# dvalcarce/filmyou-core

Hardware: AMD Instinct MI355X
Metric: top-N recs/sec (RM2), ml25m shape (higher is better)
Workload: dtype f32 (scores and logs fp32 / v_log_f32, folded in fp64; co-rating sums 64-bit fixed point in LDS (fp64 fallback); G stored as 24-bit e7m17 floats scaled per cluster above 4096 items; ratings fp16 in the row kernel when exactly representable)

## Files before the change

### filmyou-core_amd/csrc/fy_api.hip

```cpp
#include <algorithm>
#include <cstdlib>
#include <memory>
#include <mutex>
#include <new>
#include <unordered_map>

#include "fy_prep.hpp"
#include "fy_rm2.hpp"
#include "fy_ratings_update.hpp"
#include "fy_rm2_request.hpp"
#include "fy_itemsim_request.hpp"

namespace fy {
static thread_local char g_err[512] = "";
void set_error(const char* fmt, ...) {
    va_list ap;
    va_start(ap, fmt);
    vsnprintf(g_err, sizeof g_err, fmt, ap);
    va_end(ap);
}
const char* last_error() { return g_err; }
}

using namespace fy;

void fy::load_tuning_from_env(Tuning& t) {
    t = Tuning{};
    if (const char* e = getenv("FY_M24")) t.pack24 = atoi(e) != 0;
    if (const char* e = getenv("FY_M24_MIN_ITEMS")) t.pack24_min_items = std::max(0, atoi(e));
    if (const char* e = getenv("FY_SCORE_SLICES")) t.max_slices = atoi(e);
    if (const char* e = getenv("FY_SCORE_UPW")) { int v = atoi(e); if (v >= 1) t.users_per_wave = v; }
    if (const char* e = getenv("FY_PRUNE")) t.prune = atoi(e) != 0;
    if (const char* e = getenv("FY_LAZY_MIRROR")) t.lazy_mirror = atoi(e) != 0;
    if (const char* e = getenv("FY_REFINE")) t.refine = atoi(e) != 0;
    if (const char* e = getenv("FY_REFINE_C")) { double v = atof(e); if (v >= 0.0 && v < 1e6) t.refine_c = (float)v; }
    if (const char* e = getenv("FY_FULL_WALK_SPARSE")) t.full_walk_sparse = atoi(e) != 0;
    if (const char* e = getenv("FY_PREP_PACKED")) t.prep_packed = atoi(e) != 0;
    if (const char* e = getenv("FY_OVERLAP_VALUES")) t.overlap_values = atoi(e) != 0;
    if (const char* e = getenv("FY_SHARD_PREP")) t.shard_prep = atoi(e) != 0;
    if (const char* e = getenv("FY_SUP_BOUNDS")) t.sup_bounds = atoi(e) != 0;
    if (const char* e = getenv("FY_COOP")) t.coop = atoi(e) != 0;
    if (const char* e = getenv("FY_COOP_FORCE")) t.coop_force = atoi(e) != 0;
    if (const char* e = getenv("FY_COOC_PK")) t.cooc_pk = atoi(e) != 0;
    if (const char* e = getenv("FY_COOC_F32")) t.cooc_f32 = atoi(e) != 0;
    if (const char* e = getenv("FY_COOC_HALF")) t.cooc_half = atoi(e) != 0;
    if (const char* e = getenv("FY_COOC_FX")) t.cooc_fx = atoi(e) != 0;
    if (const char* e = getenv("FY_PANEL_MIN_CLUSTERS")) { int v = atoi(e); if (v >= 1) t.panel_min_clusters = v; }
    if (const char* e = getenv("FY_PANEL_COLS")) { int v = atoi(e); if (v >= 256) { t.panel_cols = v; t.panel_wide_below_users = 0; } }
    if (const char* e = getenv("FY_PANEL_WIDE_BELOW_USERS")) { int v = atoi(e); if (v >= 0) t.panel_wide_below_users = v; }
    if (const char* e = getenv("FY_PANEL_MAX_CH")) { int v = atoi(e); if (v >= 256) t.panel_max_ch = v; }
    if (const char* e = getenv("FY_BOUNDED_TABLES")) t.bounded_tables = atoi(e) != 0;
    if (const char* e = getenv("FY_COOC_PLANES")) t.cooc_planes = atoi(e) != 0;
    if (const char* e = getenv("FY_SCORE_HEAVY")) { int v = atoi(e); if (v >= 0) t.score_heavy = v; }
    if (const char* e = getenv("FY_PANEL_REPAIR")) t.panel_repair = atoi(e) != 0;
    if (const char* e = getenv("FY_PANEL_MULTI_LAUNCH")) t.panel_multi_launch = atoi(e) != 0;
    if (const char* e = getenv("FY_FLAT")) t.flat_batch = atoi(e) != 0;
    if (const char* e = getenv("FY_PANEL_SYM")) t.panel_sym = atoi(e) != 0;
    if (const char* e = getenv("FY_DEBUG_SYNC")) t.debug_sync = atoi(e);
    if (const char* e = getenv("FY_PANEL_GROUP_MB")) t.panel_group_bytes = std::max<int64_t>(0, (int64_t)atoll(e)) << 20;
    if (const char* e = getenv("FY_FLAT_BUDGET_MB")) t.flat_budget = std::max<int64_t>(0, (int64_t)atoll(e)) << 20;
    if (const char* e = getenv("FY_PANEL_TWO_PHASE")) t.panel_two_phase = atoi(e) != 0;
    if (const char* e = getenv("FY_PANEL_LANES")) { int v = atoi(e); if (v >= 1 && v <= 8) t.panel_lanes = v; }
    if (const char* e = getenv("FY_PRUNE_MIN_ITEMS")) { t.prune_min_items = atoi(e); t.prune_min_users = 0; }
    if (const char* e = getenv("FY_PRUNE_MIN_USERS")) { int v = atoi(e); if (v >= 0) t.prune_min_users = v; }
    if (const char* e = getenv("FY_SEED_CHUNKS")) { int v = atoi(e); if (v >= 0 && v <= 40) { t.seed_chunks = v; t.seed_forced = v > 0; } }
    if (const char* e = getenv("FY_WORKSPACE_GB")) { long v = atol(e); if (v >= 1) t.workspace_default = (int64_t)v << 30; }
    if (const char* e = getenv("FY_LANES")) { int v = atoi(e); if (v >= 1 && v <= 8) { t.lanes = v; t.lanes_forced = true; } }
    if (const char* e = getenv("FY_COOC_BLOCK")) { int v = atoi(e); if (v == 256 || v == 512 || v == 1024) t.cooc_block = v; }
    if (const char* e = getenv("FY_COOC_MAX_CH")) { int v = atoi(e); if (v >= 64 && v <= 20224) { t.cooc_max_ch = v; t.cooc_max_ch_forced = true; } }
    if (const char* e = getenv("FY_TOPN_FORCE_SELECT")) t.force_select = atoi(e) != 0;
    if (const char* e = getenv("FY_MAX_SURV_FRAC")) { double v = atof(e); if (v >= 0.0) t.max_surv_frac = v; }
    if (const char* e = getenv("FY_REQ_FULL_SHARE")) { double v = atof(e); if (v >= 0.0) t.req_full_share = v; }
    if (const char* e = getenv("FY_REQ_CHUNK")) { int v = atoi(e); if (v >= 64 && v <= 16384 && v % 64 == 0) t.req_chunk = v; }
    if (const char* e = getenv("FY_UPD_LDS_KEYS")) { int v = atoi(e); if (v >= 0 && v <= fy::UPD_LDS_KEYS_MAX) t.upd_lds_keys = v; }
    if (const char* e = getenv("FY_ISIM_HEAVY")) t.isim_heavy = std::max(0, atoi(e));
    if (const char* e = getenv("FY_ISIM_GRAM")) t.isim_gram = atoi(e) != 0;
    if (const char* e = getenv("FY_ISIM_GRAM_MIN_ITEMS")) t.isim_gram_min_items = std::max(0, atoi(e));
    if (const char* e = getenv("FY_ISIM_CAPG")) { int v = atoi(e); if (v >= 1 && v <= 2040) t.isim_capg = v; }
    if (const char* e = getenv("FY_ISIM_ACC32")) t.isim_acc32 = atoi(e) != 0;
    if (const char* e = getenv("FY_ISIM_PIECE")) { int v = atoi(e); if (v >= 64 && v <= 8192 && v % 64 == 0) t.isim_piece = v; }
    if (const char* e = getenv("FY_ISIM_REQ_CHUNK")) { int v = atoi(e); if (v >= 64 && v <= 16384 && v % 64 == 0) t.isim_req_chunk = v; }
    if (const char* e = getenv("FY_ISIM_REQ_ROWS")) t.isim_req_rows = std::max(0, atoi(e));
}

namespace {
std::mutex& g_jobs_mu = *new std::mutex;
std::unordered_map<const fy_rm2_job*, fy::Context*>& g_jobs = *new std::unordered_map<const fy_rm2_job*, fy::Context*>;
fy::Context* job_context(const fy_rm2_job* j) {
    std::lock_guard<std::mutex> g(g_jobs_mu);
    auto it = g_jobs.find(j);
    return it == g_jobs.end() ? nullptr : it->second;
}
inline void select_device(const fy::Context* ctx) {
    if (ctx) FY_HIP(hipSetDevice(ctx->device));
}
}

#define FY_TRY try {
#define FY_CATCH                                                           \
    }                                                                      \
    catch (const fy::Failure& f) { return f.code; }                        \
    catch (const std::bad_alloc&) {                                        \
        fy::set_error("host allocation failed");                           \
        return FY_ERR_OUT_OF_MEMORY;                                       \
    }                                                                      \
    catch (const std::exception& e) {                                      \
        fy::set_error("unexpected: %s", e.what());                         \
        return FY_ERR_HIP;                                                 \
    }                                                                      \
    return FY_OK;

extern "C" {

int fy_abi_version(void) { return FY_ABI_VERSION; }
const char* fy_last_error(void) { return fy::last_error(); }

int fy_context_create(int device_ordinal, fy_context** out) {
    if (!out) { set_error("out is NULL"); return FY_ERR_INVALID_ARGUMENT; }
    *out = nullptr;
    FY_TRY
    int n = 0;
    hipError_t e = hipGetDeviceCount(&n);
    if (e != hipSuccess || n <= 0) {
        (void)hipGetLastError();
        FY_FAIL(FY_ERR_NO_DEVICE, "no HIP device is visible (%s); this library has no CPU fallback",
                e == hipSuccess ? "device count 0" : hipGetErrorString(e));
    }
    if (device_ordinal < 0 || device_ordinal >= n) FY_FAIL(FY_ERR_INVALID_ARGUMENT, "device %d of %d", device_ordinal, n);
    FY_HIP(hipSetDevice(device_ordinal));
    hipDeviceProp_t prop;
    FY_HIP(hipGetDeviceProperties(&prop, device_ordinal));
    if (std::string(prop.gcnArchName).rfind("gfx950", 0) != 0)
        FY_FAIL(FY_ERR_NO_DEVICE, "device %d is %s; the kernels are built for gfx950 (MI355X) only", device_ordinal, prop.gcnArchName);
    std::unique_ptr<fy_context> c(new fy_context);
    c->c.device = device_ordinal;
    c->c.num_cus = prop.multiProcessorCount;
    c->c.total_mem = prop.totalGlobalMem;
    FY_HIP(hipStreamCreateWithFlags(&c->c.stream, hipStreamNonBlocking));
    fy::load_tuning_from_env(c->c.tune);
    *out = c.release();
    FY_CATCH
}

void fy_context_destroy(fy_context* c) {
    if (!c) return;
    (void)hipSetDevice(c->c.device);
    if (c->c.stream) {
        for (hipStream_t x : c->c.aux) (void)hipStreamSynchronize(x);
        (void)hipStreamSynchronize(c->c.stream);
        c->c.trim();
        for (auto& kv : c->c.capacity) (void)hipFree(kv.first);
        c->c.capacity.clear();
        for (hipStream_t x : c->c.aux) { (void)hipStreamSynchronize(x); (void)hipStreamDestroy(x); }
        (void)hipStreamDestroy(c->c.stream);
    }
    delete c;
}

int fy_context_inject_alloc_failure(fy_context* c, int64_t nth) {
    if (!c || nth < 0) { set_error("context is NULL or nth < 0"); return FY_ERR_INVALID_ARGUMENT; }
    c->c.fail_alloc_in = nth;
    return FY_OK;
}

int fy_context_reload_tuning(fy_context* c) {
    if (!c) { set_error("context is NULL"); return FY_ERR_INVALID_ARGUMENT; }
    fy::load_tuning_from_env(c->c.tune);
    return FY_OK;
}

int fy_context_synchronize(fy_context* c) {
    if (!c) { set_error("context is NULL"); return FY_ERR_INVALID_ARGUMENT; }
    FY_TRY
    select_device(&c->c);
    FY_HIP(hipStreamSynchronize(c->c.stream));
    FY_CATCH
}

void* fy_context_stream(fy_context* c) { return c ? (void*)c->c.stream : nullptr; }

int fy_ratings_create(fy_context* c, int64_t nnz, const int32_t* user, const int32_t* item, const float* score, int location,
                      fy_ratings** out) {
    if (!out) { set_error("out is NULL"); return FY_ERR_INVALID_ARGUMENT; }
    *out = nullptr;
    if (!c) { set_error("context is NULL"); return FY_ERR_INVALID_ARGUMENT; }
    if (nnz < 0 || (nnz > 0 && (!user || !item || !score))) { set_error("ratings arrays are NULL or nnz < 0"); return FY_ERR_INVALID_ARGUMENT; }
    if (location != FY_HOST && location != FY_DEVICE) { set_error("location must be FY_HOST or FY_DEVICE"); return FY_ERR_INVALID_ARGUMENT; }
    FY_TRY
    FY_HIP(hipSetDevice(c->c.device));
    std::unique_ptr<fy_ratings> r(new fy_ratings);
    r->ctx = &c->c;
    r->nnz = nnz;
    r->user.alloc(&c->c, (size_t)nnz);
    r->item.alloc(&c->c, (size_t)nnz);
    r->score.alloc(&c->c, (size_t)nnz);
    if (nnz) {
        const hipMemcpyKind k = location == FY_HOST ? hipMemcpyHostToDevice : hipMemcpyDeviceToDevice;
        FY_HIP(hipMemcpyAsync(r->user.get(), user, (size_t)nnz * 4, k, c->c.stream));
        FY_HIP(hipMemcpyAsync(r->item.get(), item, (size_t)nnz * 4, k, c->c.stream));
        FY_HIP(hipMemcpyAsync(r->score.get(), score, (size_t)nnz * 4, k, c->c.stream));
        FY_HIP(hipStreamSynchronize(c->c.stream));
        fy::ratings_id_bounds(&c->c, r.get());
    }
    *out = r.release();
    FY_CATCH
}
// ... 349 lines not shown
```

### filmyou-core_amd/csrc/fy_rm2.hip

```cpp
#include <algorithm>
#include <cmath>
#include <cstdlib>
#include <type_traits>

#include "fy_cooc.hpp"
#include "fy_prep.hpp"
#include <chrono>
#include "fy_rm2.hpp"
#include "fy_rm2_plan.hpp"
#include "fy_rm2_request.hpp"

namespace fy {

static inline int grid_for(int64_t n, int block = 256, int cap = 256 * 16) {
    int64_t g = ceil_div(n, block);
    return (int)std::max<int64_t>(1, std::min<int64_t>(g, cap));
}

constexpr int PAIR_HEAVY = 2048;
struct PairPass {
    const int32_t* __restrict__ rank_pair;
    const int32_t* __restrict__ pair_start;
    const int32_t* __restrict__ pair_di;
    const int32_t* __restrict__ csc_slot;
// ... 964 lines not shown
        }
        best = max(max(best, max(v[0], v[1])), max(v[2], v[3]));
    }
    if (Bmax_) {
        uint8_t* bp = reinterpret_cast<uint8_t*>(Bmax_) + ((int64_t)row * ldb + B) * 3;
        bp[0] = (uint8_t)best;
        bp[1] = (uint8_t)(best >> 8);
        bp[2] = (uint8_t)(best >> 16);
    }
}

__global__ __launch_bounds__(256) void k_mirror_diag(float* __restrict__ M_, int64_t ldm, int32_t Ic, float* __restrict__ Bmax_, int64_t ldb) {
    mirror_diag_body(M_, ldm, Ic, Bmax_, ldb);
}
struct PanelDesc {
    float* Gp;
    float* Bmax64;
    uint32_t* Brep;
    int64_t panel_cols, ldb64;
    int32_t Ic, p_eff, nsub, pad;
};
__global__ __launch_bounds__(1024) void k_mirror_tiles_multi(const PanelDesc* __restrict__ D) {
    const PanelDesc d = D[blockIdx.z];
    if ((int)blockIdx.x >= (int)(d.panel_cols / 128) || (int)blockIdx.y >= (int)(d.panel_cols / 256) - 1) return;
    mirror_tiles_body(d.Gp, d.panel_cols, d.p_eff, nullptr, 0);
}
__global__ __launch_bounds__(256) void k_mirror_diag_multi(const PanelDesc* __restrict__ D) {
    const PanelDesc d = D[blockIdx.y];
    if ((int)blockIdx.x >= (int)(d.panel_cols / 256)) return;
    mirror_diag_body(d.Gp, d.panel_cols, d.p_eff, nullptr, 0);
}
__global__ __launch_bounds__(256) void k_panel_colmax(const PanelDesc* __restrict__ D) {
    const PanelDesc dsc = D[blockIdx.z];
    const float* __restrict__ Gp_ = dsc.Gp;
    float* __restrict__ Bmax64_ = dsc.Bmax64;
    uint32_t* __restrict__ Brep = dsc.Brep;
    const int64_t panel_cols = dsc.panel_cols, ldb64 = dsc.ldb64;
    const int32_t Ic = dsc.Ic, p_eff = dsc.p_eff, nsub = dsc.nsub;
    if ((int)blockIdx.x * 256 >= p_eff || (int)blockIdx.y * 16 >= nsub) return;
    __shared__ uint32_t sh_m[16][257], sh_r[16][257];
    const int lane = threadIdx.x & 63, wave = threadIdx.x >> 6;
    const int col0 = blockIdx.x * 256, sbg = blockIdx.y * 16;
    const int c = col0 + 4 * lane;
    const unsigned char* __restrict__ base = reinterpret_cast<const unsigned char*>(Gp_) + (int64_t)c * 3;
    const int64_t pitch = panel_cols * 3;
    for (int s = 0; s < 4; s++) {
        const int sb = sbg + 4 * wave + s;
        uint32_t t1[4] = {0, 0, 0, 0}, t2[4] = {0, 0, 0, 0};
        if (sb < nsub) {
            const int j0 = 64 * sb, nr = min(64, Ic - j0);
            for (int r = 0; r < nr; r += 8) {
                uint32_t d[8][3];
#pragma unroll
                for (int x = 0; x < 8; x++) {
                    const uint32_t* __restrict__ p = reinterpret_cast<const uint32_t*>(base + (int64_t)(j0 + min(r + x, nr - 1)) * pitch);
                    d[x][0] = p[0]; d[x][1] = p[1]; d[x][2] = p[2];
                }
#pragma unroll
                for (int x = 0; x < 8; x++) {
                    if (r + x < nr) {
                        uint32_t v[4];
                        fy_unpack24_raw(d[x][0], d[x][1], d[x][2], v);
#pragma unroll
                        for (int q = 0; q < 4; q++) {
                            const uint32_t key = (v[q] << 6) | (uint32_t)(r + x);
                            t2[q] = max(min(t1[q], key), t2[q]);
                            t1[q] = max(t1[q], key);
                        }
                    }
                }
            }
        }
#pragma unroll
        for (int q = 0; q < 4; q++) {
            sh_m[4 * wave + s][4 * lane + q] = t1[q] >> 6;
            sh_r[4 * wave + s][4 * lane + q] = (t1[q] >> 6) ? (((t2[q] >> 6) << 8) | (t1[q] & 63u)) : 0u;
        }
    }
    __syncthreads();
    const int i = col0 + threadIdx.x;
    if (i < p_eff) {
        uint32_t m[16];
#pragma unroll
        for (int k = 0; k < 16; k++) m[k] = sh_m[k][threadIdx.x];
        uint32_t* __restrict__ bp = reinterpret_cast<uint32_t*>(reinterpret_cast<unsigned char*>(Bmax64_) + ((int64_t)i * ldb64 + sbg) * 3);
#pragma unroll
        for (int g = 0; g < 4; g++) {
            const uint32_t* v = m + 4 * g;
            bp[3 * g + 0] = v[0] | (v[1] << 24);
            bp[3 * g + 1] = (v[1] >> 8) | (v[2] << 16);
            bp[3 * g + 2] = (v[2] >> 16) | (v[3] << 8);
        }
        uint32_t* __restrict__ rp = Brep + (int64_t)i * ldb64 + sbg;
#pragma unroll
        for (int k = 0; k < 16; k++) rp[k] = sh_r[k][threadIdx.x];
    }
}

static void launch_mirror(Context* ctx, float* M, int64_t ldm, int32_t Ic, float* Bmax, int64_t ldb, hipStream_t st, const int32_t* need = nullptr,
                          int32_t write_below = 0x7FFFFFFF, bool diag = true) {
    const int nblk = (int)(ldm / 256), ntile = (int)(ldm / 128);
    if (nblk > 1) {
        FY_HIP(hipFuncSetAttribute(reinterpret_cast<const void*>(k_mirror_tiles), hipFuncAttributeMaxDynamicSharedMemorySize, 128 * MIRROR_PITCH));
        const bool split = !need && Bmax && write_below < nblk - 1;
        const int ny = split ? write_below : nblk - 1;
        if (ny > 0) {
            k_mirror_tiles<<<dim3(ntile, ny), 1024, 128 * MIRROR_PITCH, st>>>(M, ldm, Ic, Bmax, ldb, need, write_below);
            FY_KERNEL_CHECK();
        }
        if (split) {
            k_colmax_upper<<<dim3(nblk, nblk - 1 - write_below), 1024, 0, st>>>(M, ldm, Ic, Bmax, ldb, write_below);
            FY_KERNEL_CHECK();
        }
    }
    if (diag) {
        k_mirror_diag<<<nblk, 256, 0, st>>>(M, ldm, Ic, Bmax, ldb);
        FY_KERNEL_CHECK();
    }
}

static void cooc_rm2_allow_lds() {
    const int bytes = 160 * 1024 - 256;
    FY_HIP(hipFuncSetAttribute(reinterpret_cast<const void*>(k_cooc_rm2<false, double>), hipFuncAttributeMaxDynamicSharedMemorySize, bytes));
    FY_HIP(hipFuncSetAttribute(reinterpret_cast<const void*>(k_cooc_rm2<true, double>), hipFuncAttributeMaxDynamicSharedMemorySize, bytes));
    FY_HIP(hipFuncSetAttribute(reinterpret_cast<const void*>(k_cooc_rm2<false, float>), hipFuncAttributeMaxDynamicSharedMemorySize, bytes));
    FY_HIP(hipFuncSetAttribute(reinterpret_cast<const void*>(k_cooc_rm2<true, float>), hipFuncAttributeMaxDynamicSharedMemorySize, bytes));
    FY_HIP(hipFuncSetAttribute(reinterpret_cast<const void*>(k_cooc_rm2<true, unsigned long long>), hipFuncAttributeMaxDynamicSharedMemorySize, bytes));
    FY_HIP(hipFuncSetAttribute(reinterpret_cast<const void*>(k_cooc_rm2<true, uint32_t>), hipFuncAttributeMaxDynamicSharedMemorySize, bytes));
    FY_HIP(hipFuncSetAttribute(reinterpret_cast<const void*>(k_cooc_rm2<true, unsigned long long, 1>), hipFuncAttributeMaxDynamicSharedMemorySize, bytes));
    FY_HIP(hipFuncSetAttribute(reinterpret_cast<const void*>(k_cooc_rm2_multi<true, unsigned long long, 0>), hipFuncAttributeMaxDynamicSharedMemorySize, bytes));
    FY_HIP(hipFuncSetAttribute(reinterpret_cast<const void*>(k_cooc_rm2_multi<true, unsigned long long, 1>), hipFuncAttributeMaxDynamicSharedMemorySize, bytes));
}
static void stray_allow_lds();

#include "fy_rm2_kernels.hpp"

static_assert(TOPN_MAX == fy::TOPN_LIST_MAX, "fy_rm2.hpp states the top-N kernels' limit for the other translation units");
static void stray_allow_lds() {
    FY_HIP(hipFuncSetAttribute(reinterpret_cast<const void*>(k_score_stray), hipFuncAttributeMaxDynamicSharedMemorySize, (STRAY_UCAP + 1) * (int)sizeof(int32_t)));
}

void launch_topn_rows(Context* ctx, hipStream_t st, const float* S, int64_t ldS, int32_t n_cols, int32_t n_rows,
                      const int32_t* n_out, const int32_t* out_off, const int32_t* rank_item_raw, const int32_t* slot2du,
                      const int32_t* uid, int32_t slot0, int32_t aux_value, int32_t* out_user, int32_t* out_item,
                      float* out_score, int32_t* out_aux, int32_t* overflow, int32_t* any_overflow, int32_t top_n_hint) {
    if (n_rows <= 0) return;
    if (!st) st = ctx->stream;
    TopNArgs TA{S, ldS, n_cols, n_out, out_off, rank_item_raw, slot2du, uid, slot0, slot0, aux_value, out_user, out_item, out_score, out_aux,
                0, 0, nullptr, nullptr, 0, nullptr, nullptr, nullptr};
    FY_HIP(hipMemsetAsync(any_overflow, 0, sizeof(int32_t), st));
    if (top_n_hint > TOPN_LONG) k_topn_long<<<n_rows, 256, (size_t)fy_topn_long_cap(top_n_hint) * 8, st>>>(TA, overflow, any_overflow, 0, fy_topn_long_cap(top_n_hint));
    else k_topn_fast<<<n_rows, 256, 0, st>>>(TA, overflow, any_overflow, 0);
    FY_KERNEL_CHECK();
    k_topn_select<<<n_rows, 256, 0, st>>>(TA, overflow, any_overflow);
    FY_KERNEL_CHECK();
}

}

using namespace fy;

struct TableCache {
    bool valid = false;
    int64_t total_segments = 0;
    std::vector<int32_t> sig;
    bool have_x = false;
    DevBuf<float> csc_x, csc_x_over_s;
    DevBuf<uint32_t> csr_pk, y_pk;
    DevBuf<int32_t> csc_rank, samples;
    std::vector<SegTable> segs, segs_tail;
    DevBuf<int32_t> g_co, g_co_tail, g_cnt, g_ptr, g_start;
    DevBuf<int2> g_seg;
    DevBuf<float> g_w;
};
struct RM2Static {
    int32_t K = 0, rank = 0, world = 1;
    int32_t max_item = -1;
    bool has_count = false;
    std::vector<int32_t> map_user, map_cluster, cluster_count;
    Prepared P;
    int32_t slot_lo = 0, slot_hi = 0;
    DevBuf<double> partial;
    bool sharded = false;
    int64_t n_raw_users = 0, n_raw_items = 0;
    std::vector<int32_t> owner;
    DevBuf<double> partial_raw;
    int deferred_code = 0;
    std::string deferred_msg;
    int64_t exchange_len() const { return sharded ? n_raw_items + 1 + n_raw_users + 1 : (int64_t)P.nI + 1; }
    DevBuf<double> b_rank, usum_slot;
    DevBuf<long long> walk_rank;
    DevBuf<int32_t> cnt_rank, deg_slot;
    DevBuf<float> fx_rank;
    std::vector<float> fx_bounds;
    double ms_build = 0;
    TableCache tables;
    std::shared_ptr<void> request_state;
    bool matches(const fy_rm2_params* prm, int64_t n_map, const int32_t* mu, const int32_t* mc, const int32_t* cc) const {
        if (K != prm->number_of_clusters || rank != prm->rank || world != prm->world || (int64_t)map_user.size() != n_map || has_count != (cc != nullptr)) return false;
        if (n_map && (memcmp(map_user.data(), mu, (size_t)n_map * 4) || memcmp(map_cluster.data(), mc, (size_t)n_map * 4))) return false;
        if (cc && memcmp(cluster_count.data(), cc, (size_t)K * 4)) return false;
        return true;
    }
};

struct fy_rm2_job {
    Context* ctx = nullptr;
    fy_rm2_params prm{};
    std::shared_ptr<RM2Static> S;
    Prepared& P;
    int32_t &slot_lo, &slot_hi;
    DevBuf<double>& partial;
    DevBuf<double> stats;
    DevBuf<double> stats_raw;
    bool have_global = false;
    double ms_prepare = 0;
    bool from_cache = false;
    fy_collectives coll{};
    bool have_coll = false;
    DevBuf<double> gathered;
    DevBuf<double>&b_rank, &usum_slot;
    DevBuf<long long>& walk_rank;
    DevBuf<int32_t>&cnt_rank, &deg_slot;
    DevBuf<float>& fx_rank;
    std::vector<float>& fx_bounds;
    bool count_balanced = false;
    explicit fy_rm2_job(std::shared_ptr<RM2Static> s)
        : S(std::move(s)), P(S->P), slot_lo(S->slot_lo), slot_hi(S->slot_hi), partial(S->partial), b_rank(S->b_rank), usum_slot(S->usum_slot),
          walk_rank(S->walk_rank), cnt_rank(S->cnt_rank), deg_slot(S->deg_slot), fx_rank(S->fx_rank), fx_bounds(S->fx_bounds) {}
};

static void owner_range(const fy_rm2_job* J, int k, int32_t& lo, int32_t& hi) {
    if (J->S->sharded) { lo = 0; hi = k == J->prm.rank ? J->P.nU : 0; return; }
    if (!J->count_balanced) { rank_slot_range(J->P, k, J->prm.world, lo, hi); return; }
    const int64_t n = J->P.nU, W = J->prm.world;
    lo = (int32_t)(n * k / W);
    hi = (int32_t)(n * (k + 1) / W);
}

using ScoreTune = fy::Tuning;


static int cooc_item_grab(int64_t visits, int64_t n_items) { return n_items > 0 && visits / n_items < 12000 ? 8 : 1; }

static void launch_cooc_rm2(Context* ctx, const ScoreTune& tune, bool use_pk, const CoocArgs& CA_, const MEpilogue& ME, int n_items,
                            int32_t* counter, hipStream_t st) {
    if (n_items <= 0) return;
    CoocArgs CA = CA_;
    CA.acc_quarter = tune.cooc_planes ? cooc_lds_columns(CA.CH) / 4 : 0;
    const bool acc32 = CA.acc32 && use_pk && CA.fx_scale > 0.0 && !tune.cooc_f32;
    const size_t lds = (size_t)cooc_lds_columns(CA.CH) * ((tune.cooc_f32 || acc32) ? 4 : 8);
    const int by_lds = (int)std::max<size_t>(1, (160 * 1024 - 512) / (lds + 64));
    int block = tune.cooc_block;
    if (!block) block = by_lds >= 4 ? 256 : (by_lds >= 2 ? 512 : 1024);
    const int per_cu = std::max(1, std::min(by_lds, 2048 / block));
    const int grid = std::min(n_items, ctx->num_cus * per_cu);
    if (acc32) {
        k_cooc_rm2<true, uint32_t><<<grid, block, lds, st>>>(CA, ME, n_items, counter);
    } else if (use_pk && CA.fx_scale > 0.0 && !tune.cooc_f32) {
        if (ME.ceil24) k_cooc_rm2<true, unsigned long long, 1><<<grid, block, lds, st>>>(CA, ME, n_items, counter);
        else k_cooc_rm2<true, unsigned long long><<<grid, block, lds, st>>>(CA, ME, n_items, counter);
    } else if (!tune.cooc_f32) {
        if (use_pk) k_cooc_rm2<true, double><<<grid, block, lds, st>>>(CA, ME, n_items, counter);
        else k_cooc_rm2<false, double><<<grid, block, lds, st>>>(CA, ME, n_items, counter);
    } else {
        if (use_pk) k_cooc_rm2<true, float><<<grid, block, lds, st>>>(CA, ME, n_items, counter);
        else k_cooc_rm2<false, float><<<grid, block, lds, st>>>(CA, ME, n_items, counter);
    }
    FY_KERNEL_CHECK();
}

bool fy::gram_half_build(Context* ctx, const Prepared& P, const float* csc_w, const float* bounds3, float* G, int64_t ldm, double* ms_tables,
                         double* ms_walk, const float* csr_ones) {
    const ScoreTune tune = ctx->tune;
    const int32_t Ic = P.nP;
    if (P.K != 1 || (!csr_ones && (!P.ratings_fp16_exact || !P.ratings_positive)) || Ic <= 0) return false;
    int fxk = fx_exponent(bounds3);
    if (fxk < 0) return false;
    const int m = csr_ones ? 0 : P.ratings_frac_bits;
    const bool acc32 = tune.isim_acc32 && m <= 4 && (double)bounds3[2] * bounds3[2] * std::ldexp(1.0, 2 * m) < 16777216.0 &&
                       (double)bounds3[0] * bounds3[2] * std::ldexp(1.0, 2 * m) < 4294967296.0;
    if (acc32) fxk = 2 * m;
    int32_t CH, nch;
    pick_chunks(Ic, acc32 && !tune.cooc_max_ch_forced ? 2 * tune.cooc_max_ch : tune.cooc_max_ch, CH, nch);
    if (nch >= 256) return false;
    hipStream_t st = ctx->stream;
    cooc_rm2_allow_lds();
    EventTimer t_tab(ctx), t_walk(ctx);
    const size_t s0 = t_tab.begin();
    DevBuf<uint32_t> csr_pk(ctx, (size_t)P.nnz);
    k_pack_csr<<<grid_for(P.nnz), 256, 0, st>>>(0, (int32_t)P.nnz, CH, P.csr_idx.get(), csr_ones ? csr_ones : P.csr_r.get(), csr_pk.get());
    FY_KERNEL_CHECK();
    DevBuf<int32_t> co(ctx, (size_t)P.nU * (nch + 1)), csc_rank(ctx, (size_t)P.nnz);
    build_chunk_offsets(ctx, P.rowptr.get(), P.csr_idx.get(), 0, P.nU, CH, nch, co.get(), st);
    k_csc_rank<<<grid_for(P.nnz), 256, 0, st>>>(P.nnz, P.csc_pair.get(), P.pair_rank.get(), csc_rank.get());
    FY_KERNEL_CHECK();
    SegTable segs;
    DevBuf<int32_t> samples;
    build_csr_samples(ctx, P.nnz, P.csr_idx.get(), samples, st);
    build_segments(ctx, P.csc_slot.get(), csc_w, co.get(), 0, 0, (int32_t)P.nnz, nch, segs, st, csc_rank.get(), P.csr_idx.get(), CH, nullptr, 0, 0, samples.get());
    CoocArgs CA{P.rank_pair.get(), P.pair_start.get(), segs.ptr.get(), segs.seg.get(), segs.w.get(), P.csr_idx.get(), nullptr, 0, 0, Ic, CH, nch,
                0, Ic, 0, (int32_t)P.nnz, nullptr, 0, csr_pk.get(), nullptr, (uint32_t)std::min<int64_t>((int64_t)P.nnz * 4, 0xFFFFFFFFll)};
    CA.half = 1;
    CA.fx_scale = std::ldexp(1.0, fxk);
    CA.acc32 = acc32 ? 1 : 0;
    const int n_items = (int)cooc_item_count(Ic, CH, nch, true);
    DevBuf<int2> item_seg(ctx, (size_t)Ic * nch);
// ... 634 lines not shown
        build_segments(ctx, P.csc_slot.get(), tc.csc_x_over_s.get(), co, p.sbase, p.q0, p.nq, 1, tc.segs_tail[pi], ts, nullptr, nullptr, 0,
                       tc.csc_rank.get(), p.p_eff, 0);
    }
}

static void build_job_tables(fy_rm2_job* J, const JobPlan& jp, bool tables_cached, std::vector<int32_t>& csr_range, std::vector<DevBuf<int32_t>>& co_lane) {
    Context* ctx = J->ctx;
    const Prepared& P = J->P;
    hipStream_t st = ctx->stream;
    TableCache& tc = J->S->tables;
    const std::vector<Plan>& plans = jp.plans;
    if (!tables_cached) {
        tc.valid = false;
        tc.segs.clear();
        tc.segs_tail.clear();
        tc.segs.resize(plans.size());
        tc.segs_tail.resize(plans.size());
        tc.csr_pk.alloc(ctx, jp.use_pk ? (size_t)P.nnz : 1);
        tc.y_pk.alloc(ctx, jp.any_tail ? (size_t)P.nnz : 1);
        tc.csc_rank.alloc(ctx, jp.any_half ? (size_t)P.nnz : 1);
        if (jp.any_half) {
            k_csc_rank<<<grid_for(P.nnz), 256, 0, st>>>(P.nnz, P.csc_pair.get(), P.pair_rank.get(), tc.csc_rank.get());
            FY_KERNEL_CHECK();
            build_csr_samples(ctx, P.nnz, P.csr_idx.get(), tc.samples, st);
        }
    }
    csr_range.assign(2 * plans.size() + 2, 0);
    {
        std::vector<int32_t> where(2 * plans.size());
        for (size_t pi = 0; pi < plans.size(); pi++) {
            where[2 * pi] = plans[pi].sbase;
            where[2 * pi + 1] = plans[pi].sbase + plans[pi].Uc;
        }
        gather_to_host_i32(ctx, P.rowptr.get(), where, csr_range.data());
    }
    const bool all_at_once = plans.size() > 1 && !jp.any_coop;
    co_lane.resize((size_t)jp.NS);
    if (!all_at_once)
        for (auto& b : co_lane) b.alloc(ctx, jp.co_all);
    if (tables_cached) return;
    if (all_at_once) build_tables_all(ctx, P, plans, csr_range, jp.use_pk, tc, st);
    else
        for (size_t pi = 0; pi < plans.size(); pi++) build_tables(J, jp, pi, csr_range, st, co_lane[0].get());
}

struct FlatBuffers {
    DevBuf<char> flatM;
    DevBuf<float> flatS;
    DevBuf<int2> flat_seg;
    DevBuf<int32_t> flat_id, flat_ov, flat_flags, flat_cnt;
    DevBuf<CoocLaunch> d_flat_launch;
    DevBuf<FlatDesc> d_flat[2];
};
static void score_flat_batches(const ScoreShared& X, FlatBuffers& F) {
    fy_rm2_job* J = X.J;
    Context* ctx = X.J->ctx;
    const Prepared& P = X.J->P;
    fy_result* R = X.R;
    const ScoreTune& tune = *X.tune;
    const fy_rm2_params& prm = X.J->prm;
    const JobPlan& jp = *X.jp;
    hipStream_t st = ctx->stream;
    TableCache& tc = J->S->tables;
    const int32_t lo = X.lo;
    const double lambda = prm.lambda;
    constexpr int VEC = 4;
    for (size_t first = 0; first < jp.plans.size();) {
        std::vector<CoocLaunch> fb;
        std::vector<FlatDesc> fd[2];
        SyncOnUnwind fb_fd_guard(st);
        size_t m_bytes = 0, s_el = 0, i_el = 0, u_el = 0, n_flat = 0, last = first;
        int64_t batch_bytes = 0;
        for (; last < jp.plans.size(); last++) {
            const Plan& p = jp.plans[last];
            if (!p.flat) continue;
            if (n_flat && batch_bytes + flat_need(p) > jp.flat_budget) break;
            batch_bytes += flat_need(p);
            m_bytes += round_up((int64_t)p.Ic * p.ldm * (p.pack24 ? 3 : 4), 256);
            s_el += (size_t)(p.b - p.a) * p.ldm;
            i_el += (size_t)p.Ic * p.nch;
            u_el += (size_t)(p.b - p.a);
            n_flat++;
        }
        if (n_flat) {
            F.flatM.alloc(ctx, m_bytes);
            F.flatS.alloc(ctx, s_el);
            F.flat_seg.alloc(ctx, i_el);
            F.flat_id.alloc(ctx, i_el);
            F.flat_ov.alloc(ctx, u_el);
            F.flat_flags.alloc(ctx, 2 * n_flat);
            size_t m_at = 0, s_at = 0, i_at = 0, u_at = 0, k = 0;
            int max_grid[2] = {0, 0}, max_users[2] = {0, 0};
            for (size_t pi = first; pi < last; pi++) {
                const Plan& p = jp.plans[pi];
                if (!p.flat) continue;
                const int c = p.c;
                const int32_t nb = p.b - p.a;
                float* const Mc = reinterpret_cast<float*>(F.flatM.get() + m_at);
                float* const Sc = F.flatS.get() + s_at;
                CoocArgs CA{P.rank_pair.get(), P.pair_start.get(), tc.segs[pi].ptr_(), tc.segs[pi].seg_(), tc.segs[pi].w_(), P.csr_idx.get(),
                            X.csr_x, p.pbase, p.sbase, p.Ic, p.CH, p.nch, 0, p.Ic, p.q0, p.nq, nullptr, 0, X.csr_pk, nullptr,
                            (uint32_t)std::min<int64_t>((int64_t)P.nnz * 4, 0xFFFFFFFFll)};
                const int fxk = fx_exponent(&J->fx_bounds[3 * (size_t)c]);
                CA.fx_scale = std::ldexp(1.0, fxk);
                const double w2s = (1.0 - lambda) * (1.0 - lambda) * (double)X.gscale[(size_t)c];
                MEpilogue ME{Mc, p.ldm, (float)w2s, std::ldexp(w2s, -fxk), p.pack24 ? 1 : 0, nullptr, p.ldb, 0, 0, nullptr, p.ldb64, nullptr};
                const int n_items = (int)cooc_item_count(p.Ic, p.CH, p.nch, false);
                CA.item_seg = F.flat_seg.get() + i_at;
                CA.item_id = F.flat_id.get() + i_at;
                CA.item_grab = cooc_item_grab((size_t)c < P.cluster_deg2.size() ? P.cluster_deg2[c] : P.sum_deg2, n_items);
                fb.push_back(CoocLaunch{CA, ME, n_items, 0});

                const int n_chunks = (int)ceil_div(p.Ic, 64 * VEC);
                const int64_t fill = ceil_div(8 * (int64_t)ctx->num_cus, (int64_t)std::max(1, n_chunks) * (int64_t)n_flat);
                const int n_slices = (int)std::max<int64_t>(1, std::min<int64_t>(tune.max_slices, std::min<int64_t>(ceil_div(nb, 4), std::max<int64_t>(ceil_div(nb, 4 * (int64_t)tune.users_per_wave), fill))));
                FlatDesc d{};
                ScoreArgs& SA = d.SA;
                SA.M = Mc; SA.ldm = p.ldm; SA.Ic = p.Ic; SA.a_rank = X.a_rank + p.pbase; SA.b_rank = X.b_rank + p.pbase;
                SA.rb_off = P.rowptr.get() + p.sbase;
                SA.csr_idx = P.csr_idx.get(); SA.csr_e = X.csr_e; SA.csr_q = X.csr_q;
                SA.pvpi = X.pvpi; SA.n_out = X.n_out; SA.slot_lo = lo; SA.slot_base = p.sbase; SA.slot0 = p.a; SA.n_users = nb;
                SA.S = Sc; SA.ldS = p.ldm; SA.n_slices = n_slices; SA.n_chunks = n_chunks;
                d.n_heavy = F.flat_flags.get() + 2 * k;
                d.any_overflow = F.flat_flags.get() + 2 * k + 1;
                SA.n_heavy = tune.score_heavy > 0 ? d.n_heavy : nullptr;
                d.heavy_thresh = tune.score_heavy > 0 ? std::min(tune.score_heavy, 32) : 0x7FFFFFFF;
                d.TA = TopNArgs{Sc, p.ldm, p.Ic, X.n_out, X.out_off, P.rank_item_raw.get() + p.pbase, P.slot2du.get(), P.uid.get(), lo, p.a, c,
                                R->d_key0.get(), R->d_key1.get(), R->d_value.get(), R->d_aux.get(), 0, 0, nullptr, nullptr, 0, nullptr, nullptr, nullptr};
                d.overflow = F.flat_ov.get() + u_at;
                d.score_grid = n_chunks * n_slices;
                d.n_users = nb;
                const int f = p.pack24 ? 1 : 0;
                max_grid[f] = std::max(max_grid[f], d.score_grid);
                max_users[f] = std::max(max_users[f], nb);
                fd[f].push_back(d);
                m_at += (size_t)round_up((int64_t)p.Ic * p.ldm * (p.pack24 ? 3 : 4), 256);
                s_at += (size_t)nb * p.ldm;
                i_at += (size_t)p.Ic * p.nch;
                u_at += (size_t)nb;
                k++;
            }
            const size_t sp = X.t_cooc->begin(st);
            launch_cooc_rm2_multi(ctx, tune, fb, false, F.d_flat_launch, F.flat_cnt, st, true);
            X.t_cooc->end(sp, st);
            R->st.cooc_launches++;
            for (int f = 0; f < 2; f++) {
                if (fd[f].empty()) continue;
                const unsigned ny = (unsigned)fd[f].size();
                F.d_flat[f].alloc(ctx, fd[f].size());
                FY_HIP(hipMemcpyAsync(F.d_flat[f].get(), fd[f].data(), fd[f].size() * sizeof(FlatDesc), hipMemcpyHostToDevice, st));
                const size_t ss = X.t_score->begin(st);
                k_count_heavy_multi<<<(ny + 63) / 64, 64, 0, st>>>(F.d_flat[f].get(), (int32_t)ny);
                FY_KERNEL_CHECK();
                if (f) k_score_multi<4, true, 8><<<dim3((unsigned)max_grid[f], ny), 256, 0, st>>>(F.d_flat[f].get(), P.csr_idx.get(), X.csr_e, X.csr_q, X.pvpi, X.n_out);
                else k_score_multi<4, false, 8><<<dim3((unsigned)max_grid[f], ny), 256, 0, st>>>(F.d_flat[f].get(), P.csr_idx.get(), X.csr_e, X.csr_q, X.pvpi, X.n_out);
                FY_KERNEL_CHECK();
                X.t_score->end(ss, st);
                R->st.score_launches++;
                const size_t tt = X.t_topn->begin(st);
                k_topn_fast_multi<<<dim3((unsigned)max_users[f], ny), 256, 0, st>>>(F.d_flat[f].get(), tune.force_select);
                FY_KERNEL_CHECK();
                k_topn_select_multi<<<dim3((unsigned)max_users[f], ny), 256, 0, st>>>(F.d_flat[f].get(), X.prune_counters + 2);
                FY_KERNEL_CHECK();
                X.t_topn->end(tt, st);
            }
            FY_HIP(hipStreamSynchronize(st));
        }
        first = last;
    }
}

struct PanelBuf {
    DevBuf<float> Gp, Bmax64, amax64, bmax64;
    DevBuf<uint32_t> Brep;
    DevBuf<double> head32, tail32;
};
struct PanelPtrs {
    float *Gp, *Bmax64;
    uint32_t* Brep;
    float *amax64, *bmax64;
};
struct PanelSet {
    std::vector<PanelBuf> pbuf;
    std::vector<Lane> plane;
    std::vector<CoocLaunch> batch_main, batch_tail;
    DevBuf<CoocLaunch> d_batch_main, d_batch_tail;
    DevBuf<int32_t> d_cnt_main, d_cnt_tail;
    DevBuf<PanelDesc> d_panel_desc;
    std::vector<PanelDesc> hpd;
};
static void group_buffers(Context* ctx, const JobPlan& jp, int seed_chunks, const std::vector<Lane>& lanes, int grp, PanelSet& PS) {
    const std::vector<Plan>& plans = jp.plans;
    std::vector<PanelBuf>& pbuf = PS.pbuf;
    std::vector<Lane>& plane = PS.plane;
    for (size_t pi = 0; pi < plans.size(); pi++) {
        const Plan& p = plans[pi];
        if (!p.panel || jp.group_of[pi] != grp) continue;
        pbuf[pi].Gp.alloc(ctx, (size_t)p.Ic * p.panel_cols * 3 / 4 + 4);
        pbuf[pi].Bmax64.alloc(ctx, (size_t)p.Ic * p.ldb64 * 3 / 4 + 4);
        pbuf[pi].Brep.alloc(ctx, (size_t)p.Ic * p.ldb64 + 4);
        pbuf[pi].amax64.alloc(ctx, (size_t)p.ldb64);
        pbuf[pi].bmax64.alloc(ctx, (size_t)p.ldb64);
    }
    for (size_t pi = 0; pi < plans.size(); pi++) {
        const Plan& p = plans[pi];
        if (!p.panel || jp.group_of[pi] != grp) continue;
        Lane& W = plane[pi];
        const size_t nbp = (size_t)(p.b - p.a);
        const size_t seed_cols = (size_t)std::min<int64_t>(ceil_div(p.Ic, 256), seed_chunks) * 256;
        W.st = lanes[pi % jp.NS].st;
        W.M.alloc(ctx, 1); W.Bmax.alloc(ctx, 1); W.amax.alloc(ctx, 1); W.bmax.alloc(ctx, 1);
        W.Gp.alloc(ctx, 1); W.Bmax64.alloc(ctx, 1); W.Brep.alloc(ctx, 1); W.amax64.alloc(ctx, 1); W.bmax64.alloc(ctx, 1);
        W.item_seg.alloc(ctx, (size_t)p.Ic * p.nch); W.item_id.alloc(ctx, (size_t)p.Ic * p.nch);
        W.item_seg_t.alloc(ctx, (size_t)std::max(1, p.Ic - p.p_eff)); W.item_id_t.alloc(ctx, (size_t)std::max(1, p.Ic - p.p_eff));
        W.S.alloc(ctx, nbp * seed_cols);
        W.overflow.alloc(ctx, nbp);
        W.any_overflow.alloc(ctx, 1);
        W.n_heavy.alloc(ctx, 1);
        W.UB.alloc(ctx, nbp * (size_t)p.ldb64);
        W.tau.alloc(ctx, nbp);
        W.surv.alloc(ctx, nbp * (size_t)p.ldb64);
        W.surv_mask.alloc(ctx, nbp * (size_t)p.ldb64);
        W.n_quads.alloc(ctx, nbp + 1);
        W.quad_prefix.alloc(ctx, nbp + 1);
    }
}

struct LaneGuard {
    Context* ctx;
    hipEvent_t fork = nullptr;
    int32_t* pinned = nullptr;
    ~LaneGuard() {
        for (hipStream_t x : ctx->aux) (void)hipStreamSynchronize(x);
        (void)hipStreamSynchronize(ctx->stream);
        if (fork) (void)hipEventDestroy(fork);
        if (pinned) (void)hipHostFree(pinned);
    }
};

struct ClusterVisit {
    size_t pi;
    int grp, phase;
    Lane* L;
    hipStream_t ls;
    PanelPtrs PP;
    DevBuf<double>*H32, *T32;
    Lane* own;
    PanelSet* PS;
    int32_t* pinned;
};
struct ClusterNumbers {
    int fxk;
    double w2s;
    bool refine;
    int32_t head_rows;
    int64_t ld_head;
};
static ClusterNumbers cluster_numbers(const ScoreShared& X, const Plan& p) {
    const fy_rm2_job* J = X.J;
    const ScoreTune& tune = *X.tune;
    const double lambda = J->prm.lambda;
    const int c = p.c;
    ClusterNumbers N{};
    N.fxk = (X.jp->use_pk && tune.cooc_fx && !J->fx_bounds.empty()) ? fx_exponent(&J->fx_bounds[3 * (size_t)c]) : -1;
    N.w2s = (1.0 - lambda) * (1.0 - lambda) * (double)X.gscale[(size_t)c];
    N.refine = tune.refine && p.pack24 && !p.coop && N.fxk >= 0 && J->S->max_item >= 0 && J->S->max_item < (1 << 28) && p.Ic >= 8;
    N.head_rows = (int32_t)std::min<int64_t>(p.Ic & ~3, std::max<int64_t>(256, std::min<int64_t>(1024, (int64_t)tune.seed_chunks * 256)));
    N.ld_head = p.psym ? (int64_t)p.p_eff : p.ldm;
    return N;
}
static void checkpoint(const ScoreShared& X, const ClusterVisit& V, const char* what) {
    if (X.tune->debug_sync != 1) return;
    const hipError_t e = hipDeviceSynchronize();
    fprintf(stderr, "[fy] group %d/%d phase %d plan %zu (cluster %d): %s -> %s\n", V.grp, X.jp->n_groups, V.phase, V.pi, X.jp->plans[V.pi].c, what, hipGetErrorString(e));
    fflush(stderr);
}

static void build_cluster_matrix(const ScoreShared& X, const ClusterVisit& V, const ClusterNumbers& N) {
    fy_rm2_job* J = X.J;
    Context* ctx = X.J->ctx;
    const Prepared& P = X.J->P;
    fy_result* R = X.R;
    const ScoreTune& tune = *X.tune;
    const JobPlan& jp = *X.jp;
    TableCache& tc = J->S->tables;
    const size_t pi = V.pi;
    const int phase = V.phase;
    const Plan& p = jp.plans[pi];
    Lane& L = *V.L;
    hipStream_t ls = V.ls;
    const PanelPtrs& PP = V.PP;
    const int c = p.c;
    const int32_t sbase = p.sbase, pbase = p.pbase, Ic = p.Ic, CH = p.CH, nch = p.nch;
    const int64_t ldm = p.ldm;
    const bool pack24 = p.pack24;
    const int fxk = N.fxk;
    const double w2s = N.w2s;
    CoocArgs CA{P.rank_pair.get(), P.pair_start.get(), tc.segs[pi].ptr_(), tc.segs[pi].seg_(), tc.segs[pi].w_(), P.csr_idx.get(),
                X.csr_x, pbase, sbase, Ic, CH, nch, 0, Ic, p.q0, p.nq, nullptr, 0, X.csr_pk, nullptr,
                (uint32_t)std::min<int64_t>((int64_t)P.nnz * 4, 0xFFFFFFFFll)};
    CA.fx_scale = fxk >= 0 ? std::ldexp(1.0, fxk) : 0.0;
    MEpilogue ME{L.M.get(), ldm, (float)w2s, fxk >= 0 ? std::ldexp(w2s, -fxk) : 0.0,
                 pack24 ? 1 : 0, (p.prune && !p.panel) ? L.Bmax.get() : nullptr, p.ldb, 0,
                 p.panel ? p.panel_cols : 0, p.panel ? PP.Bmax64 : nullptr, p.ldb64, p.panel ? PP.Brep : nullptr};
    if (p.panel) ME.M = PP.Gp;
    if (N.refine) {
        V.H32->alloc(ctx, (size_t)N.head_rows * N.ld_head + 4);
// ... 19 lines not shown
    const bool batched = phase == 1 && tune.panel_multi_launch && jp.use_pk && fxk >= 0 && !tune.cooc_f32;
    if (p.p_eff < Ic) {
        CoocArgs CB{P.rank_pair.get(), P.pair_start.get(), tc.segs_tail[pi].ptr_(), tc.segs_tail[pi].seg_(), tc.segs_tail[pi].w_(), P.csr_idx.get(),
                    X.csr_x, pbase, sbase, Ic, p.tail_width, 1, p.p_eff, Ic - p.p_eff, p.q0, p.nq, nullptr, 0, tc.y_pk.get(), nullptr, CA.pk_bytes};
        CB.fx_scale = CA.fx_scale;
        MEpilogue MB{reinterpret_cast<float*>(reinterpret_cast<char*>(PP.Bmax64) + (size_t)(p.p_eff / 64) * 3), p.tail_width, ME.w2, ME.fx_inv, 1,
                     nullptr, 0, 0, 0, nullptr, 0, nullptr, p.ldb64, 1};
        int2* const tseg = batched ? V.own->item_seg_t.get() : L.item_seg.get();
        int32_t* const tid = batched ? V.own->item_id_t.get() : L.item_id.get();
        if (!batched) {
            k_item_list<<<grid_for((int64_t)(Ic - p.p_eff)), 256, 0, ls>>>(CB, tseg, tid);
            FY_KERNEL_CHECK();
        }
        CB.item_seg = tseg;
        CB.item_id = tid;
        CB.item_grab = 8;
        if (batched) V.PS->batch_tail.push_back(CoocLaunch{CB, MB, Ic - p.p_eff, 0});
        else {
            FY_HIP(hipMemsetAsync(L.any_overflow.get(), 0, sizeof(int32_t), ls));
            launch_cooc_rm2(ctx, tune, jp.use_pk, CB, MB, Ic - p.p_eff, L.any_overflow.get(), ls);
            R->st.cooc_launches++;
        }
        CA.tail_row0 = p.p_eff;
        CA.tail_chunks = p.tail_chunks;
    }
    {
        CA.half = (p.half || p.psym) ? 1 : 0;
        if (p.psym) { CA.half_rows = p.p_eff; CA.head_chunks = p.tail_chunks; }
        const int n_items = p.psym ? (int)(cooc_half_item_index(p.p_eff - 1, p.tail_chunks - 1, CH, p.tail_chunks) + 1 + (int64_t)(Ic - p.p_eff) * p.tail_chunks)
                            : CA.tail_chunks > 0 ? (int)((int64_t)p.p_eff * nch + (int64_t)(Ic - p.p_eff) * p.tail_chunks)
                                                 : (int)cooc_item_count(Ic, CH, nch, p.half);
        int2* const mseg = batched ? V.own->item_seg.get() : L.item_seg.get();
        int32_t* const mid = batched ? V.own->item_id.get() : L.item_id.get();
        if (!batched) {
            k_item_list<<<grid_for((int64_t)Ic * nch), 256, 0, ls>>>(CA, mseg, mid);
            FY_KERNEL_CHECK();
        }
        CA.item_seg = mseg;
        CA.item_id = mid;
        CA.item_grab = cooc_item_grab(((size_t)c < P.cluster_deg2.size() ? P.cluster_deg2[c] : P.sum_deg2) / (p.half ? 2 : 1), n_items);
        if (batched) V.PS->batch_main.push_back(CoocLaunch{CA, ME, n_items, 0});
        else {
            FY_HIP(hipMemsetAsync(L.any_overflow.get(), 0, sizeof(int32_t), ls));
            launch_cooc_rm2(ctx, tune, jp.use_pk, CA, ME, n_items, L.any_overflow.get(), ls);
        }
    }
    X.t_cooc->end(sp, ls);
    X.side->join(ls);
    checkpoint(X, V, "row kernel queued / run");
    if (!batched) R->st.cooc_launches++;
    if (p.half) {
        const size_t sm = X.t_mirror->begin(ls);
        const bool lazy = p.prune && tune.lazy_mirror;
        launch_mirror(ctx, L.M.get(), ldm, Ic, p.prune ? L.Bmax.get() : nullptr, p.ldb, ls, nullptr, lazy ? std::min(tune.seed_chunks, p.nblk) : 0x7FFFFFFF);
        X.t_mirror->end(sm, ls);
    }
    if (p.prune && !p.panel && tune.sup_bounds && !jp.long_seed) {
        const int seed_b = std::min(tune.seed_chunks, p.nblk);
        std::vector<int32_t> first;
        sup_block_map(seed_b, p.nblk, first);
        const int n_sup = (int)first.size() - 1;
        first.resize(65, first.back());
        L.sup_first.alloc(ctx, 65);
        L.Bsup.alloc(ctx, (size_t)Ic * 64);
        L.asup.alloc(ctx, 64);
        L.bsupb.alloc(ctx, 64);
        FY_HIP(hipMemcpyAsync(L.sup_first.get(), first.data(), 65 * sizeof(int32_t), hipMemcpyHostToDevice, ls));
        FY_HIP(hipStreamSynchronize(ls));
        const size_t sb = X.t_score->begin(ls);
        k_build_bsup<<<std::min<int>((Ic + 3) / 4, ctx->num_cus * 32), 256, 0, ls>>>(Ic, n_sup, L.sup_first.get(), L.Bmax.get(), p.ldb, L.Bsup.get());
        FY_KERNEL_CHECK();
        k_sup_amax<<<1, 64, 0, ls>>>(n_sup, L.sup_first.get(), L.amax.get(), L.bmax.get(), L.asup.get(), L.bsupb.get());
        FY_KERNEL_CHECK();
        X.t_score->end(sb, ls);
    }
}

static void score_cluster(const ScoreShared& X, const ClusterVisit& V, const ClusterNumbers& N) {
    fy_rm2_job* J = X.J;
    Context* ctx = X.J->ctx;
    const Prepared& P = X.J->P;
    fy_result* R = X.R;
    const ScoreTune& tune = *X.tune;
    const fy_rm2_params& prm = X.J->prm;
    const JobPlan& jp = *X.jp;
    TableCache& tc = J->S->tables;
    const size_t pi = V.pi;
    const int phase = V.phase;
    const Plan& p = jp.plans[pi];
    Lane& L = *V.L;
    hipStream_t ls = V.ls;
    const PanelPtrs& PP = V.PP;
    const int c = p.c;
    const int32_t sbase = p.sbase, pbase = p.pbase, Ic = p.Ic, a = p.a, b = p.b;
    const int64_t ldm = p.ldm;
    const bool pack24 = p.pack24;
    const int32_t lo = X.lo;
    const double lambda = prm.lambda;
    const double w2s = N.w2s;
    const bool refine = N.refine;
    const int32_t head_rows = N.head_rows;
    const int64_t ld_head = N.ld_head;
    const DevBuf<double>&H32 = *V.H32, &T32 = *V.T32;
    constexpr int VEC = 4;
    const int64_t ldS = ldm, B = p.B;
    const int n_chunks = (int)ceil_div(Ic, 64 * VEC);
    const int32_t* row_off = P.rowptr.get() + sbase;
    auto score_args = [&](const float* Mx, int64_t ldmx, int32_t Icx, const float* ax, int32_t s0, int32_t nb, float* Sx, int64_t ldSx,
                          int n_slices, int nchunks) {
        ScoreArgs SA{};
        SA.M = Mx; SA.ldm = ldmx; SA.Ic = Icx; SA.a_rank = ax; SA.b_rank = X.b_rank + pbase; SA.rb_off = row_off;
        SA.csr_idx = P.csr_idx.get(); SA.csr_e = X.csr_e; SA.csr_q = X.csr_q;
        SA.pvpi = X.pvpi; SA.n_out = X.n_out; SA.slot_lo = lo; SA.slot_base = sbase; SA.slot0 = s0; SA.n_users = nb;
        SA.S = Sx; SA.ldS = ldSx; SA.n_slices = n_slices; SA.n_chunks = nchunks;
        if (tune.score_heavy > 0) {
            const int heavy = (int64_t)nb * nchunks < 8 * (int64_t)ctx->num_cus ? std::min(tune.score_heavy, 32) : tune.score_heavy;
            k_count_heavy<<<1, 64, 0, ls>>>(P.rowptr.get() + s0, nb, heavy, L.n_heavy.get());
            SA.n_heavy = L.n_heavy.get();
        }
        return SA;
    };
    auto refine_rows = [&](int32_t s0, int32_t nb) {
        if (!refine || nb <= 0) return;
        const size_t tt = X.t_topn->begin(ls);
        const int32_t n_ids = J->S->max_item + 1;
        L.colmap.alloc(ctx, (size_t)n_ids);
        FY_HIP(hipMemsetAsync(L.colmap.get(), 0xFF, (size_t)n_ids * sizeof(int32_t), ls));
        k_refine_colmap<<<(head_rows + 255) / 256, 256, 0, ls>>>(head_rows, P.rank_item_raw.get() + pbase, L.colmap.get());
        FY_KERNEL_CHECK();
        RefineArgs RA{};
        RA.slot0 = s0; RA.n_users = nb; RA.slot_lo = lo; RA.slot_base = sbase;
        RA.n_out = X.n_out; RA.out_off = X.out_off; RA.out_item = R->d_key1.get(); RA.out_score = R->d_value.get(); RA.out_item_w = R->d_key1.get();
        RA.rowptr = P.rowptr.get(); RA.csr_idx = P.csr_idx.get(); RA.csr_r = P.csr_r.get(); RA.usum_slot = J->usum_slot.get();
        RA.p_rank = X.p_rank + pbase; RA.b_rank = X.b_rank64 + pbase;
        RA.colmap = L.colmap.get(); RA.max_item = J->S->max_item;
        RA.head_rows = head_rows;
        RA.head32 = H32.get(); RA.ld_head = ld_head; RA.tail32 = p.psym ? T32.get() : nullptr; RA.tail_from = p.p_eff;
        if (!RA.head32 || (p.psym && !RA.tail32)) FY_FAIL(FY_ERR_STATE, "internal: cluster %d has no fp32 rows for the refinement pass", c);
        RA.unscale = 1.0 / (double)X.gscale[(size_t)c];
        RA.lambda = lambda; RA.ln_items = std::log((double)prm.number_of_items); RA.ln_users = std::log((double)p.Uc);
        RA.users_minus_1 = (double)(p.Uc - 1);
        RA.refine_c = tune.refine_c;
        RA.n_refined = X.prune_counters + 5;
        int lp2 = 64;
        while (lp2 < std::min<int>(prm.number_of_recommendations, Ic)) lp2 <<= 1;
        k_refine_rows<<<(nb + 3) / 4, 256, (size_t)4 * lp2 * sizeof(uint64_t), ls>>>(RA);
        FY_KERNEL_CHECK();
        X.t_topn->end(tt, ls);
    };
    auto full_pass = [&](int32_t s0, int32_t nb, float* Sx) {
        const int n_slices = score_slices(ctx->num_cus, tune, nb, n_chunks);
        ScoreArgs SA = score_args(L.M.get(), ldm, Ic, X.a_rank + pbase, s0, nb, Sx, ldS, n_slices, n_chunks);
        const size_t ss = X.t_score->begin(ls);
        if (pack24) k_score<4, true, 8><<<n_chunks * n_slices, 256, 0, ls>>>(SA.M, SA.a_rank, SA.rb_off, SA.csr_idx, SA.csr_e, SA.csr_q, SA.pvpi, SA.n_out, SA.S, SA);
        else k_score<4, false, 8><<<n_chunks * n_slices, 256, 0, ls>>>(SA.M, SA.a_rank, SA.rb_off, SA.csr_idx, SA.csr_e, SA.csr_q, SA.pvpi, SA.n_out, SA.S, SA);
        FY_KERNEL_CHECK();
        X.t_score->end(ss, ls);
        R->st.score_launches++;
        TopNArgs TA{Sx, ldS, Ic, X.n_out, X.out_off, P.rank_item_raw.get() + pbase, P.slot2du.get(), P.uid.get(), lo, s0, c,
                    R->d_key0.get(), R->d_key1.get(), R->d_value.get(), R->d_aux.get(), 0, 0, nullptr, nullptr, 0, nullptr, nullptr, nullptr};
        const size_t tt = X.t_topn->begin(ls);
        FY_HIP(hipMemsetAsync(L.any_overflow.get(), 0, sizeof(int32_t), ls));
        if (prm.number_of_recommendations > TOPN_LONG)
            k_topn_long<<<nb, 256, (size_t)fy_topn_long_cap(prm.number_of_recommendations) * 8, ls>>>(TA, L.overflow.get(), L.any_overflow.get(), tune.force_select,
                                                                                                 fy_topn_long_cap(prm.number_of_recommendations));
        else k_topn_fast<<<nb, 256, 0, ls>>>(TA, L.overflow.get(), L.any_overflow.get(), tune.force_select);
        FY_KERNEL_CHECK();
        k_topn_select<<<nb, 256, 0, ls>>>(TA, L.overflow.get(), L.any_overflow.get(), X.prune_counters + 2);
        FY_KERNEL_CHECK();
        X.t_topn->end(tt, ls);
        refine_rows(s0, nb);
    };
    for (int32_t s0 = a; s0 < b; s0 += (int32_t)B) {
        const int32_t nb = (int32_t)std::min<int64_t>(B, b - s0);
        if (!p.prune) { full_pass(s0, nb, L.S.get()); continue; }
        const int seed_chunks = std::min(n_chunks, tune.seed_chunks);
        const bool use_sup = tune.sup_bounds && !p.panel && !jp.long_seed;
        const int n_slices = score_slices(ctx->num_cus, tune, nb, seed_chunks + (use_sup ? 0 : (int)(p.ldb / 256)));
        const bool split = jp.two_phase && p.panel && s0 == sbase && nb == p.Uc;
        if (phase == 3 && !split) continue;
        size_t ss = X.t_score->begin(ls);
        const int seed_blocks = seed_chunks;
        const int64_t SC = (int64_t)seed_chunks * 256;
        const float* Gmat = p.panel ? PP.Gp : L.M.get();
        const int64_t gld = p.panel ? (int64_t)p.panel_cols : ldm;
        const int64_t bld = p.panel ? p.ldb64 : p.ldb;
        const int bchunks = (int)(bld / 256);
        int32_t hv[3] = {0, 0, 0};
        if (phase != 3) {
        if (use_sup) {
            ScoreArgs SU = score_args(Gmat, gld, Ic, X.a_rank + pbase, s0, nb, L.S.get(), SC, n_slices, seed_chunks);
            L.UBs.alloc(ctx, (size_t)nb * 64);
            SU.Bsup = L.Bsup.get(); SU.asup = L.asup.get(); SU.bsup_b = L.bsupb.get(); SU.UBsup = L.UBs.get();
            SU.n_sup = std::min(64, std::max(0, p.nblk - seed_chunks));
            k_score_sup<<<seed_chunks * n_slices, 256, 0, ls>>>(SU.M, SU.a_rank, SU.rb_off, SU.csr_idx, SU.csr_e, SU.csr_q, SU.pvpi, SU.n_out, SU.S, SU);
            FY_KERNEL_CHECK();
        }
        ScoreArgs SA = score_args(Gmat, gld, Ic, X.a_rank + pbase, s0, nb, L.S.get(), SC, n_slices, seed_chunks + bchunks);
        SA.chunks1 = seed_chunks;
        SA.M2 = p.panel ? PP.Bmax64 : L.Bmax.get();
        SA.ldm2 = bld;
        SA.Ic2 = p.panel ? p.nsub : p.nblk;
        SA.a2 = p.panel ? PP.amax64 : L.amax.get();
        SA.b2 = p.panel ? PP.bmax64 : L.bmax.get();
        SA.S2 = L.UB.get();
        SA.ldS2 = bld;
        SA.no_mask2 = 1;
        if (!use_sup) {
            k_score<4, true, 8><<<(seed_chunks + bchunks) * n_slices, 256, 0, ls>>>(SA.M, SA.a_rank, SA.rb_off, SA.csr_idx, SA.csr_e, SA.csr_q, SA.pvpi, SA.n_out, SA.S, SA);
            FY_KERNEL_CHECK();
        }
        TopNArgs T1{L.S.get(), SC, Ic, X.n_out, X.out_off, P.rank_item_raw.get() + pbase, P.slot2du.get(), P.uid.get(),
                    lo, s0, c, R->d_key0.get(), R->d_key1.get(), R->d_value.get(), R->d_aux.get(),
                    1, seed_chunks * 256, L.surv.get(), L.n_quads.get(), bld, L.tau.get()};
        if (jp.long_seed) {
            k_topn_long<<<nb, 256, (size_t)fy_topn_long_cap(prm.number_of_recommendations) * 8, ls>>>(T1, L.overflow.get(), L.any_overflow.get(), 0,
                                                                                                 fy_topn_long_cap(prm.number_of_recommendations));
        } else {
            int lp2 = 64;
            while (lp2 < std::min<int>(std::min<int>(Ic, seed_chunks * 256), TOPN_SAMPLE)) lp2 <<= 1;
            const unsigned sg = (unsigned)((nb + 3) / 4);
            if (lp2 <= 64) k_topn_seed<1><<<sg, 256, 0, ls>>>(T1, nb, L.overflow.get());
            else if (lp2 == 128) k_topn_seed<2><<<sg, 256, 0, ls>>>(T1, nb, L.overflow.get());
            else if (lp2 == 256) k_topn_seed<4><<<sg, 256, 0, ls>>>(T1, nb, L.overflow.get());
            else if (lp2 == 512) k_topn_seed<8><<<sg, 256, 0, ls>>>(T1, nb, L.overflow.get());
            else k_topn_seed<16><<<sg, 256, 0, ls>>>(T1, nb, L.overflow.get());
        }
        FY_KERNEL_CHECK();
        FY_HIP(hipMemsetAsync(L.n_quads.get(), 0, ((size_t)nb + 1) * sizeof(int32_t), ls));
        if (p.panel)
            k_bound_select_sub<<<grid_for((int64_t)nb * 64, 256), 256, 0, ls>>>(L.UB.get(), bld, p.nsub, p.nblk, seed_blocks, L.tau.get(),
                                                                               X.pvpi + (s0 - lo), nb, bld, L.surv.get(), L.surv_mask.get(), L.n_quads.get());
        else if (use_sup)
            k_bound_select_sup<<<grid_for((int64_t)nb * 64, 256), 256, 0, ls>>>(L.UBs.get(), std::min(64, std::max(0, p.nblk - seed_chunks)), L.sup_first.get(), L.tau.get(),
                                                                               X.pvpi + (s0 - lo), nb, p.ldb, L.surv.get(), L.n_quads.get());
        else
            k_bound_select<<<grid_for((int64_t)nb * 64, 256), 256, 0, ls>>>(L.UB.get(), p.ldb, p.nblk, seed_blocks, L.tau.get(), X.pvpi + (s0 - lo), nb,
                                                                           L.surv.get(), L.n_quads.get());
        FY_KERNEL_CHECK();
        if (tune.debug_sync == 3 && !p.panel) {
            DevBuf<int32_t> cnt(ctx, (size_t)p.nblk + 1);
            FY_HIP(hipMemsetAsync(cnt.get(), 0, ((size_t)p.nblk + 1) * sizeof(int32_t), ls));
            k_surv_block_counts<<<std::min<int>(nb, 4096), 64, 0, ls>>>(nb, L.n_quads.get(), L.surv.get(), p.ldb, cnt.get());
            std::vector<int32_t> hc((size_t)p.nblk + 1);
            FY_HIP(hipMemcpyAsync(hc.data(), cnt.get(), hc.size() * sizeof(int32_t), hipMemcpyDeviceToHost, ls));
            FY_HIP(hipStreamSynchronize(ls));
            int distinct = 0;
            long long total = 0;
            for (int b2 = 0; b2 < p.nblk; b2++) { distinct += hc[b2] > 0; total += hc[b2]; }
            fprintf(stderr, "[fy] cluster %d: %lld surviving (user, block) pairs in %d distinct blocks of %d:", c, total, distinct, p.nblk);
            for (int b2 = 0; b2 < p.nblk; b2++)
                if (hc[b2]) fprintf(stderr, " %d:%d", b2, hc[b2]);
            fprintf(stderr, "\n");
        }
        if (p.panel && tune.panel_repair) {
            RepairArgs RA{L.surv.get(), L.surv_mask.get(), L.n_quads.get(), bld, nb, s0, lo, p.p_eff, Ic, P.rowptr.get(), P.csr_idx.get(),
                          X.csr_x, X.csr_e, X.csr_q, PP.Bmax64, PP.Brep, p.ldb64, PP.amax64, PP.bmax64,
                          L.tau.get(), X.pvpi, (float)w2s, X.prune_counters};
            k_bound_repair<<<std::min<int>(nb, ctx->num_cus * 16), 256, 0, ls>>>(RA);
            FY_KERNEL_CHECK();
        }
        if (p.half && !p.panel && tune.lazy_mirror) {
            const size_t sm = X.t_mirror->begin(ls);
            L.need.alloc(ctx, (size_t)p.nblk + 1);
            FY_HIP(hipMemsetAsync(L.need.get(), 0, ((size_t)p.nblk + 1) * sizeof(int32_t), ls));
            k_flag_surviving_blocks<<<std::min<int>(nb, 4096), 64, 0, ls>>>(nb, L.n_quads.get(), L.surv.get(), p.ldb, L.need.get());
            FY_KERNEL_CHECK();
            launch_mirror(ctx, L.M.get(), ldm, Ic, nullptr, p.ldb, ls, L.need.get(), 0, false);
            X.t_mirror->end(sm, ls);
        }
        exclusive_scan_i32(ctx, L.n_quads.get(), L.quad_prefix.get(), (size_t)nb + 1, ls, &L.scan_tmp);
        if (split) {
            FY_HIP(hipMemcpyAsync(&V.pinned[pi], L.quad_prefix.get() + nb, sizeof(int32_t), hipMemcpyDeviceToHost, ls));
            X.t_score->end(ss, ls);
            checkpoint(X, V, "front (seed + bound, select, second bound)");
            continue;
        }
        }
        if (!split) FY_HIP(hipMemcpyAsync(&hv[0], L.quad_prefix.get() + nb, sizeof(int32_t), hipMemcpyDeviceToHost, ls));
        else hv[0] = V.pinned[pi];
        if (s0 == sbase && nb == p.Uc) {
            hv[1] = (*X.csr_range)[2 * pi];
            hv[2] = (*X.csr_range)[2 * pi + 1];
        } else {
            FY_HIP(hipMemcpyAsync(&hv[1], P.rowptr.get() + s0, sizeof(int32_t), hipMemcpyDeviceToHost, ls));
            FY_HIP(hipMemcpyAsync(&hv[2], P.rowptr.get() + s0 + nb, sizeof(int32_t), hipMemcpyDeviceToHost, ls));
        }
        if (!split) FY_HIP(hipStreamSynchronize(ls));
        const int32_t n_surv_total = hv[0];
        const int64_t blocks_checked = (int64_t)nb * std::max(0, p.nblk - seed_blocks);
        if (!p.panel && (double)n_surv_total > tune.max_surv_frac * (double)blocks_checked) {
            X.t_score->end(ss, ls);
            if (p.half && tune.lazy_mirror) {
                const size_t sm = X.t_mirror->begin(ls);
                launch_mirror(ctx, L.M.get(), ldm, Ic, nullptr, p.ldb, ls, nullptr, 0x7FFFFFFF, false);
                X.t_mirror->end(sm, ls);
            }
            const int64_t sub = std::max<int64_t>(1, std::min<int64_t>((jp.ws / jp.NS) / (ldm * 4), nb));
            DevBuf<float> Sfull(ctx, (size_t)(sub * ldm));
            for (int32_t t0 = s0; t0 < s0 + nb; t0 += (int32_t)sub) full_pass(t0, (int32_t)std::min<int64_t>(sub, s0 + nb - t0), Sfull.get());
            FY_HIP(hipStreamSynchronize(ls));
            R->st.prune_fallbacks++;
            R->st.score_launches++;
            *X.blocks_total += blocks_checked;
            *X.fallback_survived += n_surv_total;
            *X.seed_terms_cols += (int64_t)(hv[2] - hv[1]) * (seed_chunks * 256 + p.ldb + ldm);
            continue;
        }
        L.Ssurv.alloc(ctx, (size_t)std::max(1, n_surv_total) * PRUNE_BLOCK);
        if (n_surv_total > 0) {
            ScoreArgs SQ = score_args(Gmat, gld, Ic, X.a_rank + pbase, s0, nb, L.Ssurv.get(), 0, n_slices, n_chunks);
            const int panel_blocks = p.panel ? p.panel_cols / 256 : 0x7FFFFFFF;
            k_score_blocks<8><<<std::min(n_surv_total, ctx->num_cus * 16), 256, 0, ls>>>(SQ.M, SQ.a_rank, P.rowptr.get(), SQ.csr_idx, SQ.csr_e, SQ.csr_q, SQ.pvpi,
                                                                L.quad_prefix.get(), L.surv.get(), SQ.S, SQ, bld, X.prune_counters, panel_blocks,
                                                                p.panel ? L.surv_mask.get() : nullptr);
            FY_KERNEL_CHECK();
            if (p.panel && panel_blocks < p.nblk) {
                const size_t slds = ((size_t)p.Uc + 1) * sizeof(int32_t);
                const int sgrid = std::min<int>(n_surv_total, ctx->num_cus * (int)std::max<size_t>(1, std::min<size_t>(6, (150 * 1024) / (slds + 34 * 1024))));
                L.strayT.alloc(ctx, (size_t)sgrid * STRAY_TCAP);
                L.stray_items.alloc(ctx, (size_t)n_surv_total + 1);
                FY_HIP(hipMemsetAsync(L.any_overflow.get(), 0, sizeof(int32_t), ls));
                k_stray_items<<<grid_for(nb), 256, 0, ls>>>(L.quad_prefix.get(), L.surv.get(), bld, nb, panel_blocks, L.stray_items.get(),
                                                           L.any_overflow.get());
                FY_KERNEL_CHECK();
                StrayArgs ST{L.quad_prefix.get(), L.surv.get(), L.surv_mask.get(), bld, nb, s0, lo, sbase, p.Uc, panel_blocks, Ic, pbase,
                             P.rowptr.get(), P.csr_idx.get(), X.csr_e, X.csr_q, P.rank_pair.get(), P.pair_start.get(), P.csc_slot.get(),
                             tc.csc_x.get(), X.a_rank + pbase, X.b_rank + pbase, X.pvpi,
                             (float)w2s, L.Ssurv.get(), L.strayT.get(), X.prune_counters, L.stray_items.get(),
                             L.any_overflow.get()};
                k_score_stray<<<sgrid, 256, slds, ls>>>(ST);
                FY_KERNEL_CHECK();
            }
        }
        X.t_score->end(ss, ls);
        R->st.score_launches += 2;
        *X.blocks_total += blocks_checked;
        *X.seed_terms_cols += (int64_t)(hv[2] - hv[1]) * (seed_chunks * 256 + (use_sup ? 64 : bld));
        const int32_t seed_cols_p = seed_chunks * 256;
        TopNArgs TA{L.S.get(), (int64_t)seed_cols_p, Ic, X.n_out, X.out_off, P.rank_item_raw.get() + pbase,
                    P.slot2du.get(), P.uid.get(), lo, s0, c, R->d_key0.get(), R->d_key1.get(), R->d_value.get(), R->d_aux.get(),
                    2, seed_cols_p, L.surv.get(), L.n_quads.get(), bld, L.tau.get(), L.Ssurv.get(), L.quad_prefix.get()};
        const size_t tt = X.t_topn->begin(ls);
        FY_HIP(hipMemsetAsync(L.any_overflow.get(), 0, sizeof(int32_t), ls));
        if (jp.long_seed)
            k_topn_long<<<nb, 256, (size_t)fy_topn_long_cap(prm.number_of_recommendations) * 8, ls>>>(TA, L.overflow.get(), L.any_overflow.get(), tune.force_select,
                                                                                                 fy_topn_long_cap(prm.number_of_recommendations));
        else k_topn_fast<<<nb, 256, 0, ls>>>(TA, L.overflow.get(), L.any_overflow.get(), tune.force_select);
        FY_KERNEL_CHECK();
        k_topn_select<<<nb, 256, 0, ls>>>(TA, L.overflow.get(), L.any_overflow.get(), X.prune_counters + 2);
        FY_KERNEL_CHECK();
        X.t_topn->end(tt, ls);
        refine_rows(s0, nb);
        checkpoint(X, V, "back (survivors, strays, lists)");
    }
}

static void visit_cluster(const ScoreShared& X, const ClusterVisit& V) {
    const JobPlan& jp = *X.jp;
    const Plan& p = jp.plans[V.pi];
    const Lane& L = *V.L;
    const PanelPtrs& PP = V.PP;
    checkpoint(X, V, "start");
    if (p.panel && (!PP.Gp || !PP.Bmax64 || !PP.Brep || !PP.amax64 || !PP.bmax64 || (jp.two_phase && (!L.S.get() || !L.UB.get() || !L.n_quads.get()) && V.phase != 1)))
        FY_FAIL(FY_ERR_STATE, "internal: cluster %d (plan %zu, group %d of %d, phase %d) has no panel buffers", p.c, V.pi, V.grp, jp.n_groups, V.phase);
    if (p.coop) {
        score_cluster_coop(X, p, V.ls);
        return;
    }
    const ClusterNumbers N = cluster_numbers(X, p);
    const bool do_build = !(V.phase >= 2 && p.panel), do_score = V.phase != 1;
    if (do_build) build_cluster_matrix(X, V, N);
    if (do_score) score_cluster(X, V, N);
}

static void launch_panel_batch(const ScoreShared& X, int grp, PanelSet& PS) {
    Context* ctx = X.J->ctx;
    fy_result* R = X.R;
    const ScoreTune& tune = *X.tune;
    const JobPlan& jp = *X.jp;
    hipStream_t st = ctx->stream;
    std::vector<PanelBuf>& pbuf = PS.pbuf;
    std::vector<CoocLaunch>&batch_main = PS.batch_main, &batch_tail = PS.batch_tail;
    std::vector<PanelDesc>& hpd = PS.hpd;
    DevBuf<PanelDesc>& d_panel_desc = PS.d_panel_desc;
    const size_t sp = X.t_cooc->begin(st);
    launch_cooc_rm2_multi(ctx, tune, batch_tail, true, PS.d_batch_tail, PS.d_cnt_tail, st, true);
    launch_cooc_rm2_multi(ctx, tune, batch_main, false, PS.d_batch_main, PS.d_cnt_main, st, true);
    X.t_cooc->end(sp, st);
    int max_cols = 0, max_nsub = 0;
    for (size_t pi = 0; pi < jp.plans.size(); pi++) {
        const Plan& p = jp.plans[pi];
        if (!p.psym || jp.group_of[pi] != grp) continue;
        hpd.push_back(PanelDesc{pbuf[pi].Gp.get(), pbuf[pi].Bmax64.get(), pbuf[pi].Brep.get(), p.panel_cols, p.ldb64, p.Ic, p.p_eff, p.nsub, 0});
        max_cols = std::max(max_cols, p.panel_cols);
        max_nsub = std::max(max_nsub, p.nsub);
    }
    if (!hpd.empty()) {
        for (size_t k = 0; k < hpd.size(); k++) {
            const PanelDesc& d = hpd[k];
            if (!d.Gp || !d.Bmax64 || !d.Brep || d.panel_cols <= 0 || d.panel_cols % 256 != 0 || d.p_eff != d.panel_cols || d.Ic < d.p_eff || d.nsub <= 0 ||
                d.ldb64 < d.nsub)
                FY_FAIL(FY_ERR_STATE, "internal: panel %zu of %zu of a batched mirror / column-maximum launch is unusable (Gp %p Bmax64 %p Brep %p panel_cols %d p_eff %d Ic %d nsub %d ldb64 %lld)",
                        k, hpd.size(), (const void*)d.Gp, (const void*)d.Bmax64, (const void*)d.Brep, (int)d.panel_cols, (int)d.p_eff, (int)d.Ic, (int)d.nsub, (long long)d.ldb64);
        }
        const size_t sm = X.t_mirror->begin(st);
        d_panel_desc.alloc(ctx, hpd.size());
        FY_HIP(hipMemcpyAsync(d_panel_desc.get(), hpd.data(), hpd.size() * sizeof(PanelDesc), hipMemcpyHostToDevice, st));
        const unsigned nz = (unsigned)hpd.size();
        if (max_cols / 256 > 1) {
            FY_HIP(hipFuncSetAttribute(reinterpret_cast<const void*>(k_mirror_tiles_multi), hipFuncAttributeMaxDynamicSharedMemorySize, 128 * MIRROR_PITCH));
            k_mirror_tiles_multi<<<dim3((unsigned)(max_cols / 128), (unsigned)(max_cols / 256 - 1), nz), 1024, 128 * MIRROR_PITCH, st>>>(d_panel_desc.get());
            FY_KERNEL_CHECK();
        }
        k_mirror_diag_multi<<<dim3((unsigned)(max_cols / 256), nz), 256, 0, st>>>(d_panel_desc.get());
        FY_KERNEL_CHECK();
        k_panel_colmax<<<dim3((unsigned)(max_cols / 256), (unsigned)ceil_div(max_nsub, 16), nz), 256, 0, st>>>(d_panel_desc.get());
        FY_KERNEL_CHECK();
        X.t_mirror->end(sm, st);
    }
    if (tune.debug_sync == 1) {
        const hipError_t e = hipDeviceSynchronize();
        fprintf(stderr, "[fy] group %d/%d: batched row kernels, mirror, column maxima -> %s\n", grp, jp.n_groups, hipGetErrorString(e));
        fflush(stderr);
    }
    R->st.cooc_launches += (batch_tail.empty() ? 0 : 1) + 1;
}

static void score_clusters(const ScoreShared& X, std::vector<Lane>& lanes, PanelSet& PS, LaneGuard& guard) {
    Context* ctx = X.J->ctx;
    const ScoreTune& tune = *X.tune;
    const JobPlan& jp = *X.jp;
    hipStream_t st = ctx->stream;
    std::vector<PanelBuf>& pbuf = PS.pbuf;
    std::vector<Lane>& plane = PS.plane;
    for (int grp = 0; grp < jp.n_groups; grp++) {
    if (jp.two_phase) {
        if (grp > 0) {
            for (size_t pi = 0; pi < jp.plans.size(); pi++)
                if (jp.plans[pi].panel && jp.group_of[pi] == grp - 1) { pbuf[pi] = PanelBuf(); plane[pi] = Lane(); }
        }
        group_buffers(ctx, jp, tune.seed_chunks, lanes, grp, PS);
        PS.batch_main.clear();
        PS.batch_tail.clear();
        PS.hpd.clear();
    }
    for (int phase = jp.two_phase ? 1 : 0; phase <= (jp.two_phase ? 3 : 0); phase++) {
    const auto host_t0 = std::chrono::steady_clock::now();
    struct PhaseClock {
        const std::chrono::steady_clock::time_point t0;
        int grp, phase;
        bool on;
        ~PhaseClock() {
            if (on) fprintf(stderr, "[fy] group %d phase %d: host queued for %.3f ms\n", grp, phase, std::chrono::duration<double, std::milli>(std::chrono::steady_clock::now() - t0).count());
        }
    } phase_clock{host_t0, grp, phase, tune.debug_sync != 0};
    if (phase == 3) {
        for (int l = 0; l < jp.NS; l++) FY_HIP(hipStreamSynchronize(lanes[l].st));
        FY_HIP(hipStreamSynchronize(st));
    }
    if ((phase == 0 || phase == 2) && jp.NS > 1) {
        if (guard.fork) { FY_HIP(hipEventDestroy(guard.fork)); guard.fork = nullptr; }
        FY_HIP(hipEventCreateWithFlags(&guard.fork, hipEventDisableTiming));
        FY_HIP(hipEventRecord(guard.fork, st));
        for (int l = 0; l < jp.NS; l++) FY_HIP(hipStreamWaitEvent(lanes[l].st, guard.fork, 0));
    }

    for (size_t pi = 0; pi < jp.plans.size(); pi++) {
        const Plan& p = jp.plans[pi];
        if (p.flat) continue;
        if (jp.group_of[pi] != grp) continue;
        if ((phase == 1 || phase == 3) && !p.panel) continue;
        const bool own = jp.two_phase && p.panel;
        Lane& L = phase == 1 ? lanes[0] : (own ? plane[pi] : lanes[pi % jp.NS]);
        const PanelPtrs PP = own ? PanelPtrs{pbuf[pi].Gp.get(), pbuf[pi].Bmax64.get(), pbuf[pi].Brep.get(), pbuf[pi].amax64.get(), pbuf[pi].bmax64.get()}
                                 : PanelPtrs{L.Gp.get(), L.Bmax64.get(), L.Brep.get(), L.amax64.get(), L.bmax64.get()};
        visit_cluster(X, ClusterVisit{pi, grp, phase, &L, phase == 1 ? st : L.st, PP, own ? &pbuf[pi].head32 : &L.head32, own ? &pbuf[pi].tail32 : &L.tail32,
                                      own ? &plane[pi] : nullptr, &PS, guard.pinned});
    }
    if (phase == 1 && (!PS.batch_main.empty() || !PS.batch_tail.empty())) launch_panel_batch(X, grp, PS);
    if (tune.debug_sync == 2) {
        (void)hipDeviceSynchronize();
        fprintf(stderr, "[fy] group %d phase %d: %.3f ms from its first queued operation to the drained device\n", grp, phase,
                std::chrono::duration<double, std::milli>(std::chrono::steady_clock::now() - host_t0).count());
    }
    }
    if (grp + 1 < jp.n_groups) {
        for (int l = 0; l < jp.NS; l++) FY_HIP(hipStreamSynchronize(lanes[l].st));
        FY_HIP(hipStreamSynchronize(st));
    }
    }
    if (jp.NS > 1) {
        for (int l = 0; l < jp.NS; l++) {
            hipEvent_t done;
            FY_HIP(hipEventCreateWithFlags(&done, hipEventDisableTiming));
            FY_HIP(hipEventRecord(done, lanes[l].st));
            FY_HIP(hipStreamWaitEvent(st, done, 0));
            FY_HIP(hipEventDestroy(done));
        }
    }
}

static void fill_score_stats(const ScoreShared& X, bool tables_cached, const std::vector<int32_t>& sig) {
// ... 231 lines not shown
```

### filmyou-core_amd/csrc/fy_rm2_coop.hpp

```cpp
#pragma once

static void coll_all_gather(fy_rm2_job* J, const void* send, void* recv, int64_t bytes, hipStream_t st) {
    if (!J->have_coll) {
        if (bytes) FY_HIP(hipMemcpyAsync(recv, send, (size_t)bytes, hipMemcpyDeviceToDevice, st));
        return;
    }
    const int rc = J->coll.all_gather(J->coll.user, send, recv, bytes, (void*)st);
    if (rc) FY_FAIL(FY_ERR_COLLECTIVE, "all_gather callback returned %d", rc);
}
static void coll_reduce_scatter(fy_rm2_job* J, const float* send, float* recv, int64_t count, hipStream_t st) {
    if (!J->have_coll) {
        if (count) FY_HIP(hipMemcpyAsync(recv, send, (size_t)count * sizeof(float), hipMemcpyDeviceToDevice, st));
        return;
    }
    const int rc = J->coll.reduce_scatter_f32(J->coll.user, send, recv, count, (void*)st);
    if (rc) FY_FAIL(FY_ERR_COLLECTIVE, "reduce_scatter callback returned %d", rc);
}

static void score_cluster_coop(const ScoreShared& X, const Plan& p, hipStream_t ls) {
    fy_rm2_job* J = X.J;
    Context* ctx = J->ctx;
    Prepared& P = J->P;
    fy_result* R = X.R;
    const ScoreTune& tune = *X.tune;
    const fy_rm2_params& prm = J->prm;
    const int W = prm.world, me = prm.rank;
    const int32_t Uc = p.Uc, sbase = p.sbase, pbase = p.pbase, Ic = p.Ic, CH = p.CH, nch = p.nch;
    const int64_t ldm = p.ldm, ldb = p.ldb;
    const double lambda = prm.lambda;

    std::vector<int32_t> ua(W), ub(W);
    int32_t Umax = 1;
    for (int k = 0; k < W; k++) {
        int32_t lo_k, hi_k;
        owner_range(J, k, lo_k, hi_k);
        ua[k] = std::max(lo_k, sbase);
        ub[k] = std::max(ua[k], std::min(hi_k, sbase + Uc));
        Umax = std::max(Umax, ub[k] - ua[k]);
    }
    const int32_t my_a = ua[me], n_mine = ub[me] - ua[me];

    const int32_t r0 = me, nrows = Ic > me ? (Ic - me + W - 1) / W : 0;
    std::vector<int32_t> hcnt((size_t)Ic);
    int64_t my_ratings = 0, my_walk = 0;
    {
        std::vector<long long> hw((size_t)Ic);
        FY_HIP(hipMemcpyAsync(hw.data(), J->walk_rank.get() + pbase, (size_t)Ic * sizeof(long long), hipMemcpyDeviceToHost, ls));
        FY_HIP(hipMemcpyAsync(hcnt.data(), J->cnt_rank.get() + pbase, (size_t)Ic * sizeof(int32_t), hipMemcpyDeviceToHost, ls));
        FY_HIP(hipStreamSynchronize(ls));
        for (int32_t i = r0; i < Ic; i += W) { my_ratings += hcnt[i]; my_walk += hw[i]; }
    }
    *X.coop_pair_contribs += my_walk - my_ratings;

    const int n_chunks = (int)ceil_div(Ic, 256);
    const int seed_chunks = std::min(n_chunks, tune.seed_chunks);
    const int seed_blocks = seed_chunks;
    const int64_t SC = (int64_t)seed_chunks * 256;
    const int bchunks = (int)(ldb / 256);
    DevBuf<float> Mloc(ctx, (size_t)std::max<int64_t>(1, (int64_t)nrows * ldm * 3 / 4 + 4)), Bloc(ctx, (size_t)std::max<int64_t>(1, (int64_t)nrows * ldb));
    DevBuf<float> amax(ctx, (size_t)ldb), bmax(ctx, (size_t)ldb);
    DevBuf<int32_t> n_out_all(ctx, (size_t)Uc), item_counter(ctx, 1);
    const int64_t nnz_c = (int64_t)p.nq;
    DevBuf<int32_t> my_cnt(ctx, (size_t)Uc + 1), my_rowptr(ctx, (size_t)Uc + 1), my_idx(ctx, (size_t)std::max<int64_t>(1, nnz_c));
    DevBuf<float> my_e(ctx, (size_t)std::max<int64_t>(1, nnz_c)), my_q(ctx, (size_t)std::max<int64_t>(1, nnz_c));
    DevBuf<double> pv_all(ctx, (size_t)Uc);
    DevBuf<unsigned long long> dummy(ctx, 2);
    DevBuf<float> seed_send(ctx, (size_t)((int64_t)W * Umax * SC)), seed(ctx, (size_t)((int64_t)Umax * SC));
    DevBuf<float> ub_send(ctx, (size_t)((int64_t)W * Umax * ldb)), UBsum(ctx, (size_t)((int64_t)Umax * ldb));
    DevBuf<float> tau(ctx, (size_t)Umax);
    DevBuf<uint16_t> surv(ctx, (size_t)((int64_t)Umax * ldb));
    DevBuf<int32_t> n_quads(ctx, (size_t)Umax + 1), quad_prefix(ctx, (size_t)Umax + 1), overflow(ctx, (size_t)Umax), any_overflow(ctx, 1);
    DevBuf<int32_t> counts(ctx, (size_t)W);
    const float* Mshift = Mloc.get();
    const float* Bshift = Bloc.get();

    {
        DevBuf<int32_t> co_tmp(ctx, (size_t)Uc * (nch + 1));
        SegTable seg;
        DevBuf<int2> item_seg(ctx, (size_t)std::max<int64_t>(1, (int64_t)nrows * nch));
        DevBuf<int32_t> item_id(ctx, (size_t)std::max<int64_t>(1, (int64_t)nrows * nch));
        build_chunk_offsets(ctx, P.rowptr.get(), P.csr_idx.get(), sbase, Uc, CH, nch, co_tmp.get(), ls);
        std::vector<int32_t> hls((size_t)nrows + 1, 0);
        for (int32_t i = 0; i < nrows; i++) hls[i + 1] = hls[i] + hcnt[r0 + (int64_t)i * W];
        DevBuf<int32_t> local_start(ctx, (size_t)nrows + 1), my_slot(ctx, (size_t)std::max<int64_t>(1, my_ratings));
        DevBuf<float> my_w(ctx, (size_t)std::max<int64_t>(1, my_ratings));
        FY_HIP(hipMemcpyAsync(local_start.get(), hls.data(), ((size_t)nrows + 1) * sizeof(int32_t), hipMemcpyHostToDevice, ls));
        if (nrows > 0) {
            k_gather_rows<<<grid_for((int64_t)nrows * 64, 256), 256, 0, ls>>>(r0, W, nrows, P.rank_pair.get() + pbase, P.pair_start.get(),
                                                                              local_start.get(), P.csc_slot.get(), X.csc_x, my_slot.get(), my_w.get());
            FY_KERNEL_CHECK();
        }
        build_segments(ctx, my_slot.get(), my_w.get(), co_tmp.get(), sbase, 0, (int32_t)my_ratings, nch, seg, ls);
        FY_HIP(hipMemsetAsync(Bloc.get(), 0, (size_t)std::max<int64_t>(1, (int64_t)nrows * ldb) * 3, ls));
        k_block_amax<<<grid_for(ldb), 256, 0, ls>>>(Ic, (int32_t)ldb, X.a_rank + pbase, X.b_rank + pbase, amax.get(), bmax.get());
        FY_KERNEL_CHECK();
        if (nrows > 0) {
            CoocArgs CA{P.rank_pair.get(), P.pair_start.get(), seg.ptr.get(), seg.seg.get(), seg.w.get(), P.csr_idx.get(),
                        X.csr_x, pbase, sbase, Ic, CH, nch, r0, nrows, 0, (int32_t)my_ratings, local_start.get(), W, X.csr_pk, nullptr,
                        (uint32_t)std::min<int64_t>((int64_t)P.nnz * 4, 0xFFFFFFFFll)};
            const int fxk = (X.csr_pk && tune.cooc_fx && !J->fx_bounds.empty()) ? fx_exponent(&J->fx_bounds[3 * (size_t)p.c]) : -1;
            CA.fx_scale = fxk >= 0 ? std::ldexp(1.0, fxk) : 0.0;
            const double w2s = (1.0 - lambda) * (1.0 - lambda) * (double)X.gscale[(size_t)p.c];
            MEpilogue ME{const_cast<float*>(Mshift), ldm, (float)w2s, fxk >= 0 ? std::ldexp(w2s, -fxk) : 0.0,
                         1, const_cast<float*>(Bshift), ldb, 1};
            const size_t sp = X.t_cooc->begin(ls);
            const int n_items = nrows * nch;
            k_item_list<<<grid_for(n_items), 256, 0, ls>>>(CA, item_seg.get(), item_id.get());
            FY_KERNEL_CHECK();
            CA.item_seg = item_seg.get();
            CA.item_id = item_id.get();
            FY_HIP(hipMemsetAsync(item_counter.get(), 0, sizeof(int32_t), ls));
            launch_cooc_rm2(ctx, tune, X.csr_pk != nullptr, CA, ME, n_items, item_counter.get(), ls);
            X.t_cooc->end(sp, ls);
            R->st.cooc_launches++;
        }
        FY_HIP(hipStreamSynchronize(ls));
    }

    k_my_csr_count<<<grid_for(((int64_t)Uc + 1) * 64, 256), 256, 0, ls>>>(Uc, sbase, P.rowptr.get(), P.csr_idx.get(), W, me, my_cnt.get());
    FY_KERNEL_CHECK();
    exclusive_scan_i32(ctx, my_cnt.get(), my_rowptr.get(), (size_t)Uc + 1, ls);
    k_my_csr_fill<<<grid_for((int64_t)Uc * 64, 256), 256, 0, ls>>>(Uc, sbase, P.rowptr.get(), P.csr_idx.get(), X.csr_e, X.csr_q, W, me, my_rowptr.get(),
                                                                   my_idx.get(), my_e.get(), my_q.get());
    FY_KERNEL_CHECK();
    FY_HIP(hipMemsetAsync(dummy.get(), 0, 2 * sizeof(unsigned long long), ls));
    k_user_meta<<<grid_for(Uc), 256, 0, ls>>>(sbase, sbase + Uc, P.slot2du.get(), P.uid.get(), P.ucluster.get(), P.udeg.get(),
                                               P.d_csize.get(), P.d_pcstart.get(), prm.number_of_items, prm.number_of_recommendations,
                                               prm.filter_users, X.cshift, pv_all.get(), n_out_all.get(), dummy.get());
    FY_KERNEL_CHECK();
    if (me != 0) FY_HIP(hipMemsetAsync(pv_all.get(), 0, (size_t)Uc * sizeof(double), ls));

    size_t ss = X.t_score->begin(ls);
    auto slices_for = [&](int32_t nb) { return score_slices(ctx->num_cus, tune, nb, seed_chunks + bchunks); };
    for (int k = 0; k < W; k++) {
        const int32_t nk = ub[k] - ua[k];
        if (nk <= 0) continue;
        const int ns = slices_for(nk);
        ScoreArgs SA{};
        SA.M = Mshift; SA.ldm = ldm; SA.Ic = Ic; SA.a_rank = X.a_rank + pbase; SA.b_rank = X.b_rank + pbase; SA.rb_off = my_rowptr.get();
        SA.csr_idx = my_idx.get(); SA.csr_e = my_e.get(); SA.csr_q = my_q.get(); SA.pvpi = pv_all.get(); SA.n_out = n_out_all.get(); SA.slot_lo = sbase; SA.slot_base = sbase; SA.slot0 = ua[k];
        SA.n_users = nk; SA.S = seed_send.get() + (int64_t)k * Umax * SC; SA.ldS = SC; SA.n_slices = ns; SA.n_chunks = seed_chunks + bchunks;
        SA.row_mul = W; SA.row_add = me;
        SA.chunks1 = seed_chunks;
        SA.M2 = Bshift;
        SA.ldm2 = ldb;
        SA.Ic2 = p.nblk;
        SA.a2 = amax.get();
        SA.b2 = bmax.get();
        SA.S2 = ub_send.get() + (int64_t)k * Umax * ldb;
        SA.ldS2 = ldb;
        SA.no_mask2 = 1;
        k_score<4, true, 8><<<(seed_chunks + bchunks) * ns, 256, 0, ls>>>(SA.M, SA.a_rank, SA.rb_off, SA.csr_idx, SA.csr_e, SA.csr_q, SA.pvpi, SA.n_out, SA.S, SA);
        FY_KERNEL_CHECK();
        R->st.score_launches += 2;
    }
    X.t_score->end(ss, ls);
    coll_reduce_scatter(J, seed_send.get(), seed.get(), (int64_t)Umax * SC, ls);
    coll_reduce_scatter(J, ub_send.get(), UBsum.get(), (int64_t)Umax * ldb, ls);
    ss = X.t_score->begin(ls);
    if (n_mine > 0) {
        TopNArgs T1{seed.get(), SC, Ic, X.n_out, X.out_off, P.rank_item_raw.get() + pbase, P.slot2du.get(), P.uid.get(),
                    X.lo, my_a, p.c, R->d_key0.get(), R->d_key1.get(), R->d_value.get(), R->d_aux.get(),
                    1, (int32_t)SC, surv.get(), n_quads.get(), ldb, tau.get(), nullptr, nullptr};
        k_topn_fast<<<n_mine, 256, 0, ls>>>(T1, overflow.get(), any_overflow.get(), 0);
        FY_KERNEL_CHECK();
    }
    FY_HIP(hipMemsetAsync(n_quads.get(), 0, ((size_t)Umax + 1) * sizeof(int32_t), ls));
    if (n_mine > 0) {
        k_bound_select<<<grid_for((int64_t)n_mine * 64, 256), 256, 0, ls>>>(UBsum.get(), ldb, p.nblk, seed_blocks, tau.get(), X.pvpi + (my_a - X.lo), n_mine,
                                                                            surv.get(), n_quads.get());
        FY_KERNEL_CHECK();
    }
    exclusive_scan_i32(ctx, n_quads.get(), quad_prefix.get(), (size_t)n_mine + 1, ls);
    DevBuf<int32_t> my_count(ctx, 1);
    FY_HIP(hipMemcpyAsync(my_count.get(), quad_prefix.get() + n_mine, sizeof(int32_t), hipMemcpyDeviceToDevice, ls));
    X.t_score->end(ss, ls);
    coll_all_gather(J, my_count.get(), counts.get(), sizeof(int32_t), ls);
    ss = X.t_score->begin(ls);
    std::vector<int32_t> hcounts((size_t)W);
    FY_HIP(hipMemcpyAsync(hcounts.data(), counts.get(), (size_t)W * sizeof(int32_t), hipMemcpyDeviceToHost, ls));
    FY_HIP(hipStreamSynchronize(ls));
    int32_t t_max = 0;
    for (int k = 0; k < W; k++) t_max = std::max(t_max, hcounts[k]);
    DevBuf<float> Ssurv;
    if (t_max > 0) {
        DevBuf<long long> entries(ctx, (size_t)t_max), entries_all(ctx, (size_t)W * t_max);
        DevBuf<float> Spart(ctx, (size_t)W * t_max * PRUNE_BLOCK);
        Ssurv.alloc(ctx, (size_t)t_max * PRUNE_BLOCK);
        FY_HIP(hipMemsetAsync(entries.get(), 0, (size_t)t_max * sizeof(long long), ls));
        if (n_mine > 0) {
            k_surv_entries<<<grid_for((int64_t)n_mine * 64, 256), 256, 0, ls>>>(n_mine, my_a, quad_prefix.get(), surv.get(), ldb, entries.get());
            FY_KERNEL_CHECK();
        }
        X.t_score->end(ss, ls);
        coll_all_gather(J, entries.get(), entries_all.get(), (int64_t)t_max * (int64_t)sizeof(long long), ls);
        ss = X.t_score->begin(ls);
        k_score_entries<8><<<ctx->num_cus * 8, 256, 0, ls>>>(Mshift, X.a_rank + pbase, X.b_rank + pbase, my_rowptr.get(), my_idx.get(), my_e.get(), my_q.get(), pv_all.get(),
                                                             entries_all.get(), counts.get(), W, t_max, sbase, Ic, ldm, W, me, Spart.get(),
                                                             X.prune_counters);
        FY_KERNEL_CHECK();
        R->st.score_launches++;
        X.t_score->end(ss, ls);
        coll_reduce_scatter(J, Spart.get(), Ssurv.get(), (int64_t)t_max * PRUNE_BLOCK, ls);
        ss = X.t_score->begin(ls);
        FY_HIP(hipStreamSynchronize(ls));
    }
    X.t_score->end(ss, ls);
    if (n_mine > 0 && hcounts[me] > 0) {
        const size_t tt = X.t_topn->begin(ls);
        TopNArgs TA{seed.get(), SC, Ic, X.n_out, X.out_off, P.rank_item_raw.get() + pbase, P.slot2du.get(), P.uid.get(),
                    X.lo, my_a, p.c, R->d_key0.get(), R->d_key1.get(), R->d_value.get(), R->d_aux.get(),
                    2, (int32_t)SC, surv.get(), n_quads.get(), ldb, tau.get(), Ssurv.get(), quad_prefix.get()};
        FY_HIP(hipMemsetAsync(any_overflow.get(), 0, sizeof(int32_t), ls));
        k_topn_fast<<<n_mine, 256, 0, ls>>>(TA, overflow.get(), any_overflow.get(), tune.force_select);
        FY_KERNEL_CHECK();
        k_topn_select<<<n_mine, 256, 0, ls>>>(TA, overflow.get(), any_overflow.get(), X.prune_counters + 2);
        FY_KERNEL_CHECK();
        X.t_topn->end(tt, ls);
    }
    *X.blocks_total += (int64_t)n_mine * std::max(0, p.nblk - seed_blocks);
    *X.coop_survived += (int64_t)hcounts[me];
    *X.seed_terms_cols += my_ratings * (SC + ldb);
    FY_HIP(hipStreamSynchronize(ls));
}
```

### filmyou-core_amd/csrc/fy_rm2_kernels.hpp

```cpp
#pragma once

struct ScoreArgs {
    const float* __restrict__ M;
    int64_t ldm;
    int32_t Ic;
    const float* __restrict__ a_rank;
    const float* __restrict__ b_rank;
    const int32_t* __restrict__ rb_off;
    const int32_t* __restrict__ csr_idx;
    const float* __restrict__ csr_e;
    const float* __restrict__ csr_q;
    const double* __restrict__ pvpi;
    const int32_t* __restrict__ n_out;
    int32_t slot_lo;
    int32_t slot_base;
    int32_t slot0;
    int32_t n_users;
    float* __restrict__ S;
    int64_t ldS;
    int32_t n_slices;
    int32_t n_chunks;
    int32_t no_mask;
    int32_t row_mul, row_add;
    int32_t chunks1;
    const float* __restrict__ M2;
    int64_t ldm2;
    int32_t Ic2;
    const float* __restrict__ a2;
    const float* __restrict__ b2;
    float* __restrict__ S2;
    int64_t ldS2;
    int32_t no_mask2;
    const int32_t* __restrict__ n_heavy;
    const float* __restrict__ Bsup;
    const float* __restrict__ asup;
    const float* __restrict__ bsup_b;
    float* __restrict__ UBsup;
    int32_t n_sup;
};
__global__ void k_count_heavy(const int32_t* __restrict__ rowptr , int32_t n_users, int32_t thresh,
                              int32_t* __restrict__ out) {
    if (blockIdx.x == 0 && threadIdx.x == 0) {
        int lo = 0, hi = n_users;
        while (lo < hi) { const int mid = (lo + hi) >> 1; if (rowptr[mid + 1] - rowptr[mid] > thresh) lo = mid + 1; else hi = mid; }
        *out = lo;
    }
}

__device__ __forceinline__ float fy_log2(float x) { return __builtin_amdgcn_logf(x); }
__device__ __forceinline__ void fy_logprod_step(float x, float& mant_prod, int& exp_sum) {
    mant_prod *= __builtin_amdgcn_frexp_mantf(x);
    exp_sum += __builtin_amdgcn_frexp_expf(x);
}
__device__ __forceinline__ double fy_logprod_fold(float mant_prod, int exp_sum) {
    return (double)__builtin_amdgcn_logf(mant_prod) + (double)exp_sum;
}

template <int VEC> struct VecT;
template <> struct VecT<1> { using type = float; };
template <> struct VecT<2> { using type = float2; };
template <> struct VecT<4> { using type = float4; };

struct U3 {
    uint32_t a, b, c;
};
__device__ __forceinline__ void fy_unpack24(const U3& d, float* f) {
    f[0] = __uint_as_float(__builtin_amdgcn_perm(0u, d.a, 0x0201000cu) >> (8 - FY_P24_SHIFT));
    f[1] = __uint_as_float(__builtin_amdgcn_perm(d.b, d.a, 0x0504030cu) >> (8 - FY_P24_SHIFT));
    f[2] = __uint_as_float(__builtin_amdgcn_perm(d.c, d.b, 0x0403020cu) >> (8 - FY_P24_SHIFT));
    f[3] = __uint_as_float(__builtin_amdgcn_perm(0u, d.c, 0x0302010cu) >> (8 - FY_P24_SHIFT));
}

__device__ __forceinline__ bool fy_bound_keeps(float ub, float tau, float pvpi) {
    if (!(ub == ub) || tau == INFINITY) return false;
    if (tau == -INFINITY) return true;
    const float S = fabsf(pvpi) + fabsf(ub - pvpi);
    return ub + (4e-6f * S + 1e-4f) >= tau;
}

template <int VEC, bool P24, int SB, bool SUP = false>
__device__ __forceinline__ void score_body(const float* __restrict__ M_, const float* __restrict__ a_rank_,
                                           const int32_t* __restrict__ rb_off_, const int32_t* __restrict__ csr_idx_,
                                           const float* __restrict__ csr_e_, const float* __restrict__ csr_q_,
                                           const double* __restrict__ pvpi_,
                                           const int32_t* __restrict__ n_out_, float* __restrict__ S_, const ScoreArgs& A, const int bx ) {
    using V = typename VecT<VEC>::type;
    using G = typename std::conditional<P24, U3, V>::type;
    static_assert(!P24 || VEC == 4, "24-bit rows are packed four columns to three dwords");
    constexpr int CW = 64 * VEC;
    const int lane = threadIdx.x & 63;
    const int wave = __builtin_amdgcn_readfirstlane(threadIdx.x >> 6);
    int chunk = bx / A.n_slices;
    const int slice = bx - chunk * A.n_slices;
    const bool second = A.chunks1 > 0 && chunk >= A.chunks1;
    if (second) chunk -= A.chunks1;
    const float* __restrict__ Msel = second ? A.M2 : M_;
    const float* __restrict__ asel = second ? A.a2 : a_rank_;
    const float* __restrict__ bsel = second ? A.b2 : A.b_rank;
    float* __restrict__ Ssel = second ? A.S2 : S_;
    const int64_t ldm_sel = second ? A.ldm2 : A.ldm, ldS_sel = second ? A.ldS2 : A.ldS;
    const int Ic_sel = second ? A.Ic2 : A.Ic, no_mask = second ? A.no_mask2 : A.no_mask;
    const int col0 = chunk * CW;
    const int col = col0 + lane * VEC;
    float a[VEC], bb[VEC];
#pragma unroll
    for (int v = 0; v < VEC; v++) {
        a[v] = col + v < Ic_sel ? asel[col + v] : 0.0f;
        bb[v] = col + v < Ic_sel ? bsel[col + v] : 0.0f;
    }
    const bool sup_here = SUP && chunk == 0 && !second;
    float as_ = 0.f, bs_ = 0.f;
    if constexpr (SUP) {
        if (sup_here && lane < A.n_sup) { as_ = A.asup[lane]; bs_ = A.bsup_b[lane]; }
    }
    const float* __restrict__ Bsup_lane = SUP ? A.Bsup + lane : nullptr;
    const char* __restrict__ Mcol = reinterpret_cast<const char*>(Msel) + (int64_t)col * (P24 ? 3 : 4);
    const int64_t pitch = ldm_sel * (P24 ? 3 : 4);
    const double LN2 = 0.69314718055994530942;
    const float qnan = __builtin_nanf("");
    const int row_mul = A.row_mul ? A.row_mul : 1;
    auto walk = [&](int beg, int end, double* t, unsigned& mask, double& ts) __attribute__((always_inline)) {
        if (beg >= end) return;
        static_assert(SB <= 64, "one lane per row of a batch");
        const int sub = lane & (SB - 1);
        int vi, vi_n;
        float ve, vq, ve_n, vq_n;
        {
            const int kk = min(beg + sub, end - 1);
            vi = csr_idx_[kk]; ve = csr_e_[kk]; vq = csr_q_[kk];
        }
        for (int k = beg; k < end; k += SB) {
            G g[SB];
            float e[SB], qq[SB];
            int jj[SB];
            float gs[SUP ? SB : 1];
#pragma unroll
            for (int q = 0; q < SB; q++) {
                jj[q] = __builtin_amdgcn_readlane(vi, q);
                e[q] = __uint_as_float(__builtin_amdgcn_readlane(__float_as_uint(ve), q));
                qq[q] = __uint_as_float(__builtin_amdgcn_readlane(__float_as_uint(vq), q));
                g[q] = *reinterpret_cast<const G*>(Mcol + (int64_t)jj[q] * pitch);
                if constexpr (SUP) {
                    if (sup_here) gs[q] = Bsup_lane[(int64_t)jj[q] * 64];
                }
            }
            {
                const int kk = min(k + SB + sub, end - 1);
                vi_n = csr_idx_[kk]; ve_n = csr_e_[kk]; vq_n = csr_q_[kk];
            }
            float p[VEC];
            int pe[VEC];
#pragma unroll
            for (int v = 0; v < VEC; v++) { p[v] = 1.f; pe[v] = 0; }
            float ps = 1.f;
            int pes = 0;
#pragma unroll
            for (int q = 0; q < SB; q++) {
                if (k + q < end) {
                    if constexpr (SUP) {
                        if (sup_here) fy_logprod_step(fmaf(qq[q], bs_, fmaf(as_, e[q], gs[q])), ps, pes);
                    }
                    float gv[VEC];
                    if constexpr (P24) fy_unpack24(g[q], gv);
                    else {
                        const float* gp = reinterpret_cast<const float*>(&g[q]);
#pragma unroll
                        for (int v = 0; v < VEC; v++) gv[v] = gp[v];
                    }
#pragma unroll
                    for (int v = 0; v < VEC; v++) fy_logprod_step(fmaf(qq[q], bb[v], fmaf(a[v], e[q], gv[v])), p[v], pe[v]);
                    const unsigned d = (unsigned)(jj[q] * row_mul + A.row_add - col0);
                    if (!no_mask && d < (unsigned)CW && (int)(d / VEC) == lane) mask |= 1u << (d % VEC);
                }
            }
#pragma unroll
            for (int v = 0; v < VEC; v++) t[v] += fy_logprod_fold(p[v], pe[v]);
            if constexpr (SUP) {
                if (sup_here) ts += fy_logprod_fold(ps, pes);
            }
            vi = vi_n; ve = ve_n; vq = vq_n;
        }
    };
    auto store = [&](int u, int slot, const double* t, unsigned mask) __attribute__((always_inline)) {
        V o;
        float* ov = reinterpret_cast<float*>(&o);
        const double base = pvpi_[slot - A.slot_lo];
#pragma unroll
        for (int v = 0; v < VEC; v++) ov[v] = (float)(base + LN2 * t[v]);
#pragma unroll
        for (int v = 0; v < VEC; v++)
            if ((mask >> v) & 1u || col + v >= Ic_sel) ov[v] = qnan;
        *reinterpret_cast<V*>(Ssel + (int64_t)u * ldS_sel + col) = o;
    };
    auto store_sup = [&](int u, int slot, double ts) __attribute__((always_inline)) {
        if constexpr (SUP) {
            if (sup_here) A.UBsup[(int64_t)u * 64 + lane] = lane < A.n_sup ? (float)(pvpi_[slot - A.slot_lo] + LN2 * ts) : qnan;
        }
    };
    __shared__ double sh_t[3][64][VEC];
    __shared__ double sh_ts[SUP ? 3 : 1][64];
    __shared__ unsigned sh_mask[3][64];
    const int n_heavy = A.n_heavy ? min(*A.n_heavy, A.n_users) : 0;
    for (int u = slice; u < n_heavy; u += A.n_slices) {
        const int slot = A.slot0 + u;
        if (n_out_[slot - A.slot_lo] == 0) continue;
        const int32_t* __restrict__ ro = rb_off_ + (slot - A.slot_base);
        const int beg = ro[0], end = ro[1];
        const int quarter = (((end - beg + 3) >> 2) + SB - 1) / SB * SB;
        const int wb = min(end, beg + wave * quarter), we = min(end, wb + quarter);
        double t[VEC];
#pragma unroll
        for (int v = 0; v < VEC; v++) t[v] = 0.0;
        unsigned mask = 0;
        double ts = 0.0;
        walk(wb, we, t, mask, ts);
        if (wave > 0) {
#pragma unroll
            for (int v = 0; v < VEC; v++) sh_t[wave - 1][lane][v] = t[v];
            sh_mask[wave - 1][lane] = mask;
            if constexpr (SUP) sh_ts[wave - 1][lane] = ts;
        }
        __syncthreads();
        if (wave == 0) {
            for (int x = 0; x < 3; x++) {
#pragma unroll
                for (int v = 0; v < VEC; v++) t[v] += sh_t[x][lane][v];
                mask |= sh_mask[x][lane];
                if constexpr (SUP) ts += sh_ts[x][lane];
            }
            store(u, slot, t, mask);
            store_sup(u, slot, ts);
        }
        __syncthreads();
    }
    for (int u = n_heavy + slice * 4 + wave; u < A.n_users; u += A.n_slices * 4) {
        const int slot = A.slot0 + u;
        if (n_out_[slot - A.slot_lo] == 0) continue;
        const int32_t* __restrict__ ro = rb_off_ + (slot - A.slot_base);
        const int beg = ro[0], end = ro[1];
        double t[VEC];
#pragma unroll
        for (int v = 0; v < VEC; v++) t[v] = 0.0;
        unsigned mask = 0;
        double ts = 0.0;
        walk(beg, end, t, mask, ts);
        store(u, slot, t, mask);
        store_sup(u, slot, ts);
    }
}
template <int VEC, bool P24, int SB>
__global__ __launch_bounds__(256) void k_score(const float* __restrict__ M_, const float* __restrict__ a_rank_,
                                               const int32_t* __restrict__ rb_off_, const int32_t* __restrict__ csr_idx_,
                                               const float* __restrict__ csr_e_, const float* __restrict__ csr_q_,
                                               const double* __restrict__ pvpi_,
                                               const int32_t* __restrict__ n_out_, float* __restrict__ S_, ScoreArgs A) {
    score_body<VEC, P24, SB>(M_, a_rank_, rb_off_, csr_idx_, csr_e_, csr_q_, pvpi_, n_out_, S_, A, (int)blockIdx.x);
}

__global__ __launch_bounds__(256) void k_score_sup(const float* __restrict__ M_, const float* __restrict__ a_rank_,
                                                   const int32_t* __restrict__ rb_off_, const int32_t* __restrict__ csr_idx_,
                                                   const float* __restrict__ csr_e_, const float* __restrict__ csr_q_,
                                                   const double* __restrict__ pvpi_,
                                                   const int32_t* __restrict__ n_out_, float* __restrict__ S_, ScoreArgs A) {
    score_body<4, true, 8, true>(M_, a_rank_, rb_off_, csr_idx_, csr_e_, csr_q_, pvpi_, n_out_, S_, A, (int)blockIdx.x);
}

struct TopNArgs {
    const float* __restrict__ S;
    int64_t ldS;
    int32_t Ic;
    const int32_t* __restrict__ n_out;
    const int32_t* __restrict__ out_off;
    const int32_t* __restrict__ rank_item_raw;
    const int32_t* __restrict__ slot2du;
    const int32_t* __restrict__ uid;
    int32_t slot_lo, slot0, cluster;
    int32_t* __restrict__ out_user;
    int32_t* __restrict__ out_item;
    float* __restrict__ out_score;
    int32_t* __restrict__ out_cluster;
    int32_t mode;
    int32_t seed_cols;
    const uint16_t* __restrict__ surv;
    const int32_t* __restrict__ n_quads;
    int64_t ldb;
    float* __restrict__ tau;
    const float* __restrict__ Ssurv;
    const int32_t* __restrict__ quad_prefix;
};

__device__ __forceinline__ uint32_t fy_order_key(float f) {
    const uint32_t b = __float_as_uint(f);
    return (b & 0x80000000u) ? ~b : (b | 0x80000000u);
}
__device__ __forceinline__ float fy_order_unkey(uint32_t k) {
    const uint32_t b = (k & 0x80000000u) ? (k & 0x7FFFFFFFu) : ~k;
    return __uint_as_float(b);
}

constexpr int TOPN_MAX = 2048;
constexpr int TOPN_CAP = 4096;
constexpr int TOPN_BINS = 4096;
constexpr int TOPN_SAMPLE = 1024;
constexpr int TOPN_LONG = 256;
constexpr int PRUNE_BLOCK_COLS = 256;
constexpr int SEED_CHUNKS_MAX = 40;

__device__ __forceinline__ void fy_bitonic_desc(uint64_t* v, int P2) {
    for (int k = 2; k <= P2; k <<= 1) {
        for (int j = k >> 1; j > 0; j >>= 1) {
            for (int i = threadIdx.x; i < P2; i += blockDim.x) {
                const int l = i ^ j;
                if (l > i) {
                    const uint64_t x = v[i], y = v[l];
                    const bool desc = (i & k) == 0;
                    if (desc ? (x < y) : (x > y)) { v[i] = y; v[l] = x; }
                }
            }
            __syncthreads();
        }
    }
}

__device__ __forceinline__ void topn_fast_body(const TopNArgs& A, int32_t* __restrict__ overflow, int32_t* __restrict__ any_overflow,
                                               int force_select, const int u ) {
    __shared__ uint64_t cand[TOPN_MAX];
    __shared__ uint32_t sh_count, sh_nvalid;
    const int slot = A.slot0 + u;
    const int K = A.n_out[slot - A.slot_lo];
    if (threadIdx.x == 0) overflow[u] = 0;
    if (A.mode == 2 && A.n_quads[u] == 0) return;
    if (K == 0) {
        if (A.mode == 1 && threadIdx.x == 0) A.tau[u] = INFINITY;
        return;
    }
    if (force_select && A.mode != 1) {
        if (threadIdx.x == 0) { overflow[u] = 1; atomicAdd(any_overflow, 1); }
        return;
    }
    const float* __restrict__ row = A.S + (int64_t)u * A.ldS;
    const int tid = threadIdx.x;
    constexpr int sample0 = TOPN_SAMPLE;
    const int Ls = min(A.Ic, A.mode ? min(A.seed_cols, TOPN_SAMPLE) : sample0);
    if (tid == 0) sh_nvalid = 0;
    __syncthreads();
    int myvalid = 0;
    int LP2 = 64;
    while (LP2 < Ls) LP2 <<= 1;
    for (int i = tid; i < LP2; i += blockDim.x) {
        uint64_t c = 0ull;
        if (i < Ls) {
            const float f = row[i];
            if (f == f) { c = ((uint64_t)fy_order_key(f) << 32) | (uint32_t)(0x7FFFFFFF - A.rank_item_raw[i]); myvalid++; }
        }
        cand[i] = c;
    }
    if (myvalid) atomicAdd(&sh_nvalid, (uint32_t)myvalid);
    __syncthreads();
    fy_bitonic_desc(cand, LP2);
    const int nvalid = (int)sh_nvalid;
    const uint32_t tau = nvalid >= K ? (uint32_t)(cand[K - 1] >> 32) : 0u;
    const int keep = min(K, nvalid);
    if (A.mode == 1) {
        if (tid == 0) A.tau[u] = nvalid >= K ? fy_order_unkey(tau) : -INFINITY;
        const int off1 = A.out_off[slot - A.slot_lo];
        const int user1 = A.uid[A.slot2du[slot]];
        for (int i = tid; i < keep; i += blockDim.x) {
            const uint64_t c = cand[i];
            A.out_user[off1 + i] = user1;
            A.out_item[off1 + i] = 0x7FFFFFFF - (int32_t)(uint32_t)c;
            A.out_score[off1 + i] = fy_order_unkey((uint32_t)(c >> 32));
            A.out_cluster[off1 + i] = A.cluster;
        }
        return;
    }
    __syncthreads();
    if (tid == 0) sh_count = (uint32_t)keep;
    __syncthreads();
    const int i4_begin = A.mode == 2 ? 0 : (sample0 >> 2);
    const int i4_end = A.mode == 2 ? A.n_quads[u] * (PRUNE_BLOCK_COLS / 4) : (A.Ic + 3) >> 2;
    auto take4 = [&](const float4& f4, int i4) __attribute__((always_inline)) {
        const float fv[4] = {f4.x, f4.y, f4.z, f4.w};
#pragma unroll
        for (int q = 0; q < 4; q++) {
            const float f = fv[q];
            const int i = 4 * i4 + q;
            if (f == f && i < A.Ic) {
                const uint32_t key = fy_order_key(f);
                if (key >= tau) {
                    const uint32_t pos = atomicAdd(&sh_count, 1u);
                    if (pos < (uint32_t)TOPN_MAX) cand[pos] = ((uint64_t)key << 32) | (uint32_t)(0x7FFFFFFF - A.rank_item_raw[i]);
                }
            }
        }
    };
    if (A.mode == 2) {
        for (int x = i4_begin + tid; x < i4_end; x += blockDim.x) {
            const unsigned blk = A.surv[(int64_t)u * A.ldb + (x >> 6)];
            const int i4 = (int)blk * (PRUNE_BLOCK_COLS / 4) + (x & 63);
            const float* src = A.Ssurv ? A.Ssurv + ((int64_t)(A.quad_prefix[u] + (x >> 6)) * PRUNE_BLOCK_COLS + 4 * (x & 63)) : row + 4 * (int64_t)i4;
            take4(*reinterpret_cast<const float4*>(src), i4);
        }
    } else {
        constexpr int UNR = 4;
        const float4 nan4 = make_float4(__builtin_nanf(""), __builtin_nanf(""), __builtin_nanf(""), __builtin_nanf(""));
        for (int x0 = i4_begin + tid; x0 < i4_end; x0 += UNR * (int)blockDim.x) {
            float4 f4[UNR];
#pragma unroll
            for (int q = 0; q < UNR; q++) {
                const int x = x0 + q * (int)blockDim.x;
                f4[q] = x < i4_end ? *reinterpret_cast<const float4*>(row + 4 * (int64_t)x) : nan4;
            }
#pragma unroll
            for (int q = 0; q < UNR; q++) take4(f4[q], x0 + q * (int)blockDim.x);
        }
    }
    __syncthreads();
// ... 258 lines not shown
        const uint64_t c = cand[i];
        A.out_user[off + i] = user_raw;
        A.out_item[off + i] = 0x7FFFFFFF - (int32_t)(uint32_t)c;
        A.out_score[off + i] = fy_order_unkey((uint32_t)(c >> 32));
        A.out_cluster[off + i] = A.cluster;
    }
}

__device__ __forceinline__ void topn_select_body(const TopNArgs& A, const int32_t* __restrict__ overflow,
                                                 const int32_t* __restrict__ any_overflow, unsigned long long* __restrict__ n_selected, const int u) {
    __shared__ uint32_t hist[TOPN_BINS];
    __shared__ uint64_t cand[TOPN_MAX];
    __shared__ uint32_t sh_prefix, sh_need, sh_count, sh_eq_taken;
    if (*any_overflow == 0) return;
    if (overflow[u] == 0) return;
    const int slot = A.slot0 + u;
    const int K = A.n_out[slot - A.slot_lo];
    if (K == 0) return;
    const float* __restrict__ row = A.S + (int64_t)u * A.ldS;
    const int tid = threadIdx.x;
    if (tid == 0 && n_selected) atomicAdd(n_selected, 1ull);
    __shared__ uint32_t live[2048];
    __shared__ uint16_t live_pre[2048];
    if (A.mode) {
        for (int w = tid; w < 2048; w += blockDim.x) live[w] = 0;
        __syncthreads();
        for (int k = tid; k < A.n_quads[u]; k += blockDim.x) {
            const unsigned blk = A.surv[(int64_t)u * A.ldb + k];
            atomicOr(&live[blk >> 5], 1u << (blk & 31u));
        }
        __syncthreads();
        if (A.Ssurv && tid == 0) {
            unsigned run = 0;
            for (int w = 0; w < 2048; w++) { live_pre[w] = (uint16_t)run; run += __popc(live[w]); }
        }
        __syncthreads();
    }
    const float* __restrict__ packed = (A.mode && A.Ssurv) ? A.Ssurv + (int64_t)A.quad_prefix[u] * PRUNE_BLOCK_COLS : nullptr;
    auto rowval = [&](int i) -> float {
        if (A.mode == 0 || i < A.seed_cols) return row[i];
        const unsigned blk = (unsigned)i >> 8, w = blk >> 5, bit = blk & 31u;
        if (!((live[w] >> bit) & 1u)) return __builtin_nanf("");
        if (!packed) return row[i];
        const unsigned pos = live_pre[w] + __popc(live[w] & ((1u << bit) - 1u));
        return packed[(int64_t)pos * PRUNE_BLOCK_COLS + (i & 255)];
    };
#define FY_ROWVAL(i) rowval(i)

    uint32_t prefix = 0, prefix_mask = 0, need = (uint32_t)K;
    const int shifts[3] = {20, 10, 0};
    const int widths[3] = {12, 10, 10};
    for (int pass = 0; pass < 3; pass++) {
        const int nb = 1 << widths[pass];
        for (int b = tid; b < nb; b += blockDim.x) hist[b] = 0;
        __syncthreads();
        for (int i = tid; i < A.Ic; i += blockDim.x) {
            const float f = FY_ROWVAL(i);
            if (f != f) continue;
            const uint32_t key = fy_order_key(f);
            if ((key & prefix_mask) == prefix) atomicAdd(&hist[(key >> shifts[pass]) & (nb - 1)], 1u);
        }
        __syncthreads();
        if (tid == 0) {
            uint32_t cum = 0;
            int b = nb - 1;
            for (; b > 0; b--) {
                if (cum + hist[b] >= need) break;
                cum += hist[b];
            }
            sh_prefix = prefix | ((uint32_t)b << shifts[pass]);
            sh_need = need - cum;
        }
        __syncthreads();
        prefix = sh_prefix;
        need = sh_need;
        prefix_mask |= (uint32_t)(nb - 1) << shifts[pass];
        __syncthreads();
    }
    const uint32_t T = prefix;
    const uint32_t eq_total = hist[T & 1023u];
    const bool take_all_eq = (eq_total == need);
    __syncthreads();

    if (tid == 0) { sh_count = 0; sh_eq_taken = 0; }
    __syncthreads();
    for (int i = tid; i < A.Ic; i += blockDim.x) {
        const float f = FY_ROWVAL(i);
        if (f != f) continue;
        const uint32_t key = fy_order_key(f);
        if (key > T || (take_all_eq && key == T)) {
            const uint32_t pos = atomicAdd(&sh_count, 1u);
            if (pos < (uint32_t)TOPN_MAX) cand[pos] = ((uint64_t)key << 32) | (uint32_t)(0x7FFFFFFF - A.rank_item_raw[i]);
        }
    }
    __syncthreads();
    if (!take_all_eq) {
        uint32_t* wave_cnt = hist;
        const int w = tid >> 6, ln = tid & 63, nw = blockDim.x >> 6;
        for (int base = 0; base < A.Ic; base += blockDim.x) {
            const int i = base + tid;
            bool eq = false;
            if (i < A.Ic) {
                const float f = FY_ROWVAL(i);
                eq = (f == f) && fy_order_key(f) == T;
            }
            const unsigned long long bal = __ballot(eq);
            if (ln == 0) wave_cnt[w] = (uint32_t)__popcll(bal);
            __syncthreads();
            uint32_t off = sh_eq_taken, all = 0;
            for (int x = 0; x < nw; x++) {
                if (x < w) off += wave_cnt[x];
                all += wave_cnt[x];
            }
            off += (uint32_t)__popcll(bal & ((1ull << ln) - 1ull));
            if (eq && off < need) {
                const uint32_t pos = atomicAdd(&sh_count, 1u);
                if (pos < (uint32_t)TOPN_MAX) cand[pos] = ((uint64_t)T << 32) | (uint32_t)(0x7FFFFFFF - A.rank_item_raw[i]);
            }
            __syncthreads();
            if (tid == 0) sh_eq_taken += all;
            __syncthreads();
            if (sh_eq_taken >= need) break;
        }
        __syncthreads();
    }
    const int n = min((int)sh_count, K);
    int P2 = 1;
    while (P2 < n) P2 <<= 1;
    for (int i = n + tid; i < P2; i += blockDim.x) cand[i] = 0ull;
    __syncthreads();
    for (int k = 2; k <= P2; k <<= 1) {
        for (int j = k >> 1; j > 0; j >>= 1) {
            for (int i = tid; i < P2; i += blockDim.x) {
                const int l = i ^ j;
                if (l > i) {
                    const uint64_t x = cand[i], y = cand[l];
                    const bool desc = (i & k) == 0;
                    if (desc ? (x < y) : (x > y)) { cand[i] = y; cand[l] = x; }
                }
            }
            __syncthreads();
        }
    }
    const int off = A.out_off[slot - A.slot_lo];
    const int user_raw = A.uid[A.slot2du[slot]];
    for (int i = tid; i < n; i += blockDim.x) {
        const uint64_t c = cand[i];
        A.out_user[off + i] = user_raw;
        A.out_item[off + i] = 0x7FFFFFFF - (int32_t)(uint32_t)c;
        A.out_score[off + i] = fy_order_unkey((uint32_t)(c >> 32));
        A.out_cluster[off + i] = A.cluster;
    }
}
__global__ __launch_bounds__(256) void k_topn_select(TopNArgs A, const int32_t* __restrict__ overflow,
                                                     const int32_t* __restrict__ any_overflow, unsigned long long* __restrict__ n_selected = nullptr) {
    topn_select_body(A, overflow, any_overflow, n_selected, (int)blockIdx.x);
}

struct FlatDesc {
    ScoreArgs SA;
    TopNArgs TA;
    int32_t* overflow;
    int32_t* any_overflow;
    int32_t* n_heavy;
    int32_t score_grid, n_users, heavy_thresh, pad;
};
__global__ void k_count_heavy_multi(const FlatDesc* __restrict__ D, int32_t n) {
    const int i = blockIdx.x * blockDim.x + threadIdx.x;
    if (i >= n) return;
    const FlatDesc& d = D[i];
    const int32_t* __restrict__ rowptr = d.SA.rb_off + (d.SA.slot0 - d.SA.slot_base);
    int lo = 0, hi = d.n_users;
    while (lo < hi) { const int mid = (lo + hi) >> 1; if (rowptr[mid + 1] - rowptr[mid] > d.heavy_thresh) lo = mid + 1; else hi = mid; }
    *d.n_heavy = lo;
    *d.any_overflow = 0;
}
template <int VEC, bool P24, int SB>
__global__ __launch_bounds__(256) void k_score_multi(const FlatDesc* __restrict__ D, const int32_t* __restrict__ csr_idx_,
                                                     const float* __restrict__ csr_e_, const float* __restrict__ csr_q_,
                                                     const double* __restrict__ pvpi_, const int32_t* __restrict__ n_out_) {
    const FlatDesc& d = D[blockIdx.y];
    if ((int)blockIdx.x >= d.score_grid) return;
    const ScoreArgs A = d.SA;
    score_body<VEC, P24, SB>(A.M, A.a_rank, A.rb_off, csr_idx_, csr_e_, csr_q_, pvpi_, n_out_, A.S, A, (int)blockIdx.x);
}
__global__ __launch_bounds__(256) void k_topn_fast_multi(const FlatDesc* __restrict__ D, int force_select) {
    const FlatDesc& d = D[blockIdx.y];
    if ((int)blockIdx.x >= d.n_users) return;
    const TopNArgs A = d.TA;
    topn_fast_body(A, d.overflow, d.any_overflow, force_select, (int)blockIdx.x);
}
__global__ __launch_bounds__(256) void k_topn_select_multi(const FlatDesc* __restrict__ D, unsigned long long* __restrict__ n_selected) {
    const FlatDesc& d = D[blockIdx.y];
    if ((int)blockIdx.x >= d.n_users) return;
    const TopNArgs A = d.TA;
    topn_select_body(A, d.overflow, d.any_overflow, n_selected, (int)blockIdx.x);
}

constexpr int PRUNE_BLOCK = 256;

__global__ void k_block_amax(int32_t Ic, int32_t ldb, const float* __restrict__ a_rank, const float* __restrict__ b_rank,
                             float* __restrict__ amax, float* __restrict__ bmax, int32_t width = PRUNE_BLOCK) {
    for (int32_t b = blockIdx.x * blockDim.x + threadIdx.x; b < ldb; b += gridDim.x * blockDim.x) {
        float m = 0.0f, mb = 0.0f;
        for (int64_t i = (int64_t)b * width; i < min((int64_t)Ic, (int64_t)(b + 1) * width); i++) { m = fmaxf(m, a_rank[i]); mb = fmaxf(mb, b_rank[i]); }
        amax[b] = m;
        bmax[b] = mb;
    }
}

template <int SB>
__global__ __launch_bounds__(256) void k_score_blocks(const float* __restrict__ M_, const float* __restrict__ a_rank_,
                                                      const int32_t* __restrict__ rowptr_, const int32_t* __restrict__ csr_idx_,
                                                      const float* __restrict__ csr_e_, const float* __restrict__ csr_q_,
                                                      const double* __restrict__ pvpi_,
                                                      const int32_t* __restrict__ surv_prefix_, const uint16_t* __restrict__ surv_,
                                                      float* __restrict__ S_, ScoreArgs A, int64_t ldb,
                                                      unsigned long long* __restrict__ counters, int32_t panel_blocks = 0x7FFFFFFF,
                                                      const uint8_t* __restrict__ surv_mask_ = nullptr) {
    __shared__ double sh_t[3][64][4];
    __shared__ unsigned sh_mask[3][64];
    const int lane = threadIdx.x & 63;
    const int wave = __builtin_amdgcn_readfirstlane((int)(threadIdx.x >> 6));
    const int total = surv_prefix_[A.n_users];
    const int64_t pitch = A.ldm * 3;
    const double LN2 = 0.69314718055994530942;
    const float qnan = __builtin_nanf("");
    unsigned long long my_terms = 0;
    if (blockIdx.x == 0 && threadIdx.x == 0 && total) atomicAdd(&counters[0], (unsigned long long)total);
    for (int w = blockIdx.x; w < total; w += gridDim.x) {
        int lo = 0, hi = A.n_users;
        while (hi - lo > 1) {
            const int mid = (lo + hi) >> 1;
            if (surv_prefix_[mid] <= w) lo = mid; else hi = mid;
        }
        const int u = lo;
        const int slot = A.slot0 + u;
        const int blk = (int)surv_[(int64_t)u * ldb + (w - surv_prefix_[u])];
        if (blk >= panel_blocks) continue;
        const bool live = !surv_mask_ || ((surv_mask_[(int64_t)u * ldb + (w - surv_prefix_[u])] >> (lane >> 4)) & 1u);
        const int col0 = blk * PRUNE_BLOCK;
        const int col = col0 + lane * 4;
        float a[4], bb[4];
#pragma unroll
        for (int v = 0; v < 4; v++) {
            a[v] = col + v < A.Ic ? a_rank_[col + v] : 0.0f;
            bb[v] = col + v < A.Ic ? A.b_rank[col + v] : 0.0f;
        }
        const char* __restrict__ Mcol = reinterpret_cast<const char*>(M_) + (int64_t)col * 3;
        const int row_beg = rowptr_[slot], row_end = rowptr_[slot + 1];
        const int quarter = (((row_end - row_beg + 3) >> 2) + SB - 1) / SB * SB;
        const int beg = min(row_end, row_beg + wave * quarter), end = min(row_end, beg + quarter);
        double t[4] = {0.0, 0.0, 0.0, 0.0};
        unsigned mask = 0;
        const int sub = lane & (SB - 1);
        int vi = 0, vi_n;
        float ve = 0.f, vq = 0.f, ve_n, vq_n;
        if (beg < end) {
            const int kk = min(beg + sub, end - 1);
            vi = csr_idx_[kk]; ve = csr_e_[kk]; vq = csr_q_[kk];
        }
        for (int k = beg; k < end; k += SB) {
            U3 g[SB];
            float e[SB], qq[SB];
            int jj[SB];
#pragma unroll
            for (int x = 0; x < SB; x++) {
                jj[x] = __builtin_amdgcn_readlane(vi, x);
                e[x] = __uint_as_float(__builtin_amdgcn_readlane(__float_as_uint(ve), x));
                qq[x] = __uint_as_float(__builtin_amdgcn_readlane(__float_as_uint(vq), x));
                g[x] = U3{0u, 0u, 0u};
                if (live) g[x] = *reinterpret_cast<const U3*>(Mcol + (int64_t)jj[x] * pitch);
            }
            {
                const int kk = min(k + SB + sub, end - 1);
                vi_n = csr_idx_[kk]; ve_n = csr_e_[kk]; vq_n = csr_q_[kk];
            }
            float p[4] = {1.f, 1.f, 1.f, 1.f};
            int pe[4] = {0, 0, 0, 0};
#pragma unroll
            for (int x = 0; x < SB; x++) {
                if (k + x < end) {
                    float gv[4];
                    fy_unpack24(g[x], gv);
#pragma unroll
                    for (int v = 0; v < 4; v++) fy_logprod_step(fmaf(qq[x], bb[v], fmaf(a[v], e[x], gv[v])), p[v], pe[v]);
                    const unsigned d = (unsigned)(jj[x] - col);
                    if (d < 4u) mask |= 1u << d;
                }
            }
#pragma unroll
            for (int v = 0; v < 4; v++) t[v] += fy_logprod_fold(p[v], pe[v]);
            vi = vi_n; ve = ve_n; vq = vq_n;
        }
        if (wave > 0) {
#pragma unroll
            for (int v = 0; v < 4; v++) sh_t[wave - 1][lane][v] = t[v];
            sh_mask[wave - 1][lane] = mask;
        }
        __syncthreads();
        if (wave == 0) {
            for (int x = 0; x < 3; x++) {
#pragma unroll
                for (int v = 0; v < 4; v++) t[v] += sh_t[x][lane][v];
                mask |= sh_mask[x][lane];
            }
            const double base = pvpi_[slot - A.slot_lo];
            float4 o;
            o.x = (!live || (mask & 1u) || col + 0 >= A.Ic) ? qnan : (float)(base + LN2 * t[0]);
            o.y = (!live || (mask & 2u) || col + 1 >= A.Ic) ? qnan : (float)(base + LN2 * t[1]);
            o.z = (!live || (mask & 4u) || col + 2 >= A.Ic) ? qnan : (float)(base + LN2 * t[2]);
            o.w = (!live || (mask & 8u) || col + 3 >= A.Ic) ? qnan : (float)(base + LN2 * t[3]);
            *reinterpret_cast<float4*>(S_ + (int64_t)w * PRUNE_BLOCK + lane * 4) = o;
            my_terms += (unsigned long long)(row_end - row_beg) * 256ull;
        }
        __syncthreads();
    }
    if (wave == 0 && lane == 0 && my_terms) atomicAdd(&counters[1], my_terms);
}

__global__ __launch_bounds__(256) void k_bound_select_sub(const float* __restrict__ UB64, int64_t ldb64, int32_t nsub, int32_t nblk, int32_t seed_blocks,
                                                          const float* __restrict__ tau, const double* __restrict__ pvpi ,
                                                          int32_t n_users, int64_t ldsurv, uint16_t* __restrict__ surv, uint8_t* __restrict__ surv_mask,
                                                          int32_t* __restrict__ n_surv) {
    const int lane = threadIdx.x & 63;
    const int wpb = blockDim.x >> 6;
    for (int u = blockIdx.x * wpb + (threadIdx.x >> 6); u < n_users; u += gridDim.x * wpb) {
        const float t = tau[u];
        const float pv = (float)pvpi[u];
        int count = 0;
        for (int b0 = 0; b0 < nblk; b0 += 64) {
            const int b = b0 + lane;
            unsigned keep = 0;
            if (b < nblk && b >= seed_blocks) {
#pragma unroll
                for (int q = 0; q < 4; q++) {
                    const int sb = 4 * b + q;
                    if (sb < nsub && fy_bound_keeps(UB64[(int64_t)u * ldb64 + sb], t, pv)) keep |= 1u << q;
                }
            }
            const unsigned long long bal = __ballot(keep != 0);
            if (keep) {
                const int64_t at = (int64_t)u * ldsurv + count + __popcll(bal & ((1ull << lane) - 1ull));
                surv[at] = (uint16_t)b;
                surv_mask[at] = (uint8_t)keep;
            }
            count += __popcll(bal);
        }
        if (lane == 0) n_surv[u] = count;
    }
}

constexpr int REPAIR_MAX_LIST = 256;
struct RepairArgs {
    uint16_t* __restrict__ surv;
    uint8_t* __restrict__ surv_mask;
    int32_t* __restrict__ n_surv;
    int64_t ldsurv;
    int32_t n_users, slot0, slot_lo, p_eff, Ic;
    const int32_t* __restrict__ rowptr;
    const int32_t* __restrict__ csr_idx;
    const float* __restrict__ csr_x;
    const float* __restrict__ csr_e;
    const float* __restrict__ csr_q;
    const float* __restrict__ Bmax64;
    const uint32_t* __restrict__ Brep;
    int64_t ldb64;
    const float* __restrict__ amax64;
    const float* __restrict__ bmax64;
    const float* __restrict__ tau;
    const double* __restrict__ pvpi;
    float w2;
    unsigned long long* __restrict__ counters;
};
__device__ __forceinline__ float fy_load24(const float* __restrict__ base3, int64_t entry) {
    const uint8_t* __restrict__ b = reinterpret_cast<const uint8_t*>(base3) + entry * 3;
    const uint32_t v = (uint32_t)b[0] | ((uint32_t)b[1] << 8) | ((uint32_t)b[2] << 16);
    return __uint_as_float(v << FY_P24_SHIFT);
}
__global__ __launch_bounds__(256) void k_bound_repair(RepairArgs A) {
    __shared__ uint8_t sh_newmask[1024];
    const int lane = threadIdx.x & 63, wave = threadIdx.x >> 6;
    const double LN2 = 0.69314718055994530942;
    unsigned long long dropped = 0;
    for (int u = blockIdx.x; u < A.n_users; u += gridDim.x) {
        const int ns = A.n_surv[u];
        const int slot = A.slot0 + u;
        const int r0 = A.rowptr[slot], r1 = A.rowptr[slot + 1];
        if (ns == 0 || r1 - r0 > REPAIR_MAX_LIST) continue;
        uint16_t* __restrict__ mine = A.surv + (int64_t)u * A.ldsurv;
        uint8_t* __restrict__ mask_of = A.surv_mask + (int64_t)u * A.ldsurv;
        const float t = A.tau[u];
        const double base = A.pvpi[slot - A.slot_lo];
        for (int k0 = 0; k0 < ns; k0 += 1024) {
            const int nk = min(1024, ns - k0);
            for (int k = k0 + wave; k < k0 + nk; k += 4) {
                const int blk = (int)mine[k];
                unsigned mask = mask_of[k];
                for (int qb = 0; qb < 4; qb++) {
                    if (!((mask >> qb) & 1u)) continue;
                    const int sb = 4 * blk + qb;
                    const int c0 = sb * 64;
                    float ymax = 0.f;
                    for (int f = r0 + lane; f < r1; f += 64) {
                        const unsigned d = (unsigned)(A.csr_idx[f] - c0);
                        if (d < 64u) ymax = fmaxf(ymax, A.csr_x[f]);
                    }
                    for (int o = 32; o > 0; o >>= 1) ymax = fmaxf(ymax, __shfl_xor(ymax, o, 64));
                    if (ymax == 0.f) continue;
                    const float am = A.amax64[sb], bm = A.bmax64[sb];
                    double sum = 0.0;
                    for (int f = r0 + lane; f < r1; f += 64) {
                        const int j = A.csr_idx[f];
                        float g = fy_load24(A.Bmax64, (int64_t)j * A.ldb64 + sb);
                        if (g > 0.f) {
                            if (j >= A.p_eff && c0 >= A.p_eff) {
                                g = fmaxf(0.f, g - A.w2 * A.csr_x[f] * ymax * 0.999999f);
                            } else {
                                const uint32_t rep = A.Brep[(int64_t)j * A.ldb64 + sb];
                                const int col = c0 + (int)(rep & 63u);
                                int l = r0, h = r1;
                                while (l < h) { const int m = (l + h) >> 1; if (A.csr_idx[m] < col) l = m + 1; else h = m; }
                                if (l < r1 && A.csr_idx[l] == col) g = __uint_as_float((rep >> 8) << FY_P24_SHIFT);
                            }
                        }
                        sum += (double)fy_log2(fmaf(A.csr_q[f], bm, fmaf(am, A.csr_e[f], g)));
                    }
                    for (int o = 32; o > 0; o >>= 1) sum += __shfl_xor(sum, o, 64);
                    if (!fy_bound_keeps((float)(base + LN2 * sum), t, (float)base)) { mask &= ~(1u << qb); dropped++; }
                }
                if (lane == 0) sh_newmask[k - k0] = (uint8_t)mask;
            }
            __syncthreads();
            if (wave == 0) {
                int kept = k0 == 0 ? 0 : A.n_surv[u];
                for (int kk = 0; kk < nk; kk += 64) {
                    const int k = kk + lane;
                    const unsigned m = k < nk ? sh_newmask[k] : 0u;
                    const int blk = k < nk ? (int)mine[k0 + k] : 0;
                    const unsigned long long bal = __ballot(m != 0u);
                    if (m) {
// ... 572 lines not shown
```

### filmyou-core_amd/csrc/fy_tuning.hpp

```cpp
#pragma once
#include <cstdint>

namespace fy {

struct Tuning {
    int force_select = 0;
    int pack24 = 1;
    int pack24_min_items = 4096;
    int max_slices = 65536;
    int users_per_wave = 16;
    int64_t workspace_default = (int64_t)16 << 30;
    int lanes = 4;
    bool lanes_forced = false;
    int prune = 1;
    int prune_min_items = 8192;
    int seed_chunks = 0;
    int cooc_block = 0;
    int cooc_max_ch = 19968;
    bool cooc_max_ch_forced = false;
    int sup_bounds = 1;
    int prep_packed = 1;
    int overlap_values = 1;
    int shard_prep = 1;
    int full_walk_sparse = 1;
    int refine = 1;
    float refine_c = 2.0f;
    int lazy_mirror = 1;
    int seed_forced = 0;
    int coop = 1;
    int coop_force = 0;
    int cooc_pk = 1;
    int cooc_f32 = 0;
    int cooc_half = 1;
    int cooc_fx = 1;
    int panel_min_clusters = 4;
    int prune_min_users = 600;
    int panel_wide_below_users = 2500;
    int panel_cols = 4096;
    bool bounded_tables = true;
    bool cooc_planes = true;
    int score_heavy = 512;
    bool panel_repair = true;
    int panel_lanes = 2;
    int64_t flat_budget = 0;
    int64_t panel_group_bytes = 0;
    int debug_sync = 0;
    bool panel_sym = true;
    bool flat_batch = true;
    bool panel_multi_launch = true;
    bool panel_two_phase = true;
    int panel_max_ch = 4096;
    double max_surv_frac = 0.25;
    double req_full_share = 1.0;
    int req_chunk = 8192;
    int upd_lds_keys = 4096;
    int isim_heavy = 4096;
    int isim_gram = -1;
    int isim_gram_min_items = 4096;
    int isim_capg = 2040;
    int isim_piece = 4096;
    int isim_acc32 = 1;
    int isim_req_chunk = 8192;
    int isim_req_rows = 0;
};

inline int64_t ceil_div(int64_t a, int64_t b) { return (a + b - 1) / b; }
inline int64_t round_up(int64_t a, int64_t b) { return ceil_div(a, b) * b; }

}
```

Measured before the change: 397.5 million.

## Add scalar-load rating walk for 24-bit score kernels and persistent top-N select grid

```diff
diff --git a/filmyou-core_amd/csrc/fy_api.hip b/filmyou-core_amd/csrc/fy_api.hip
--- a/filmyou-core_amd/csrc/fy_api.hip
+++ b/filmyou-core_amd/csrc/fy_api.hip
@@ -52,6 +52,7 @@
     if (const char* e = getenv("FY_BOUNDED_TABLES")) t.bounded_tables = atoi(e) != 0;
     if (const char* e = getenv("FY_COOC_PLANES")) t.cooc_planes = atoi(e) != 0;
     if (const char* e = getenv("FY_SCORE_HEAVY")) { int v = atoi(e); if (v >= 0) t.score_heavy = v; }
+    if (const char* e = getenv("FY_SCORE_WALK")) t.score_walk = atoi(e) != 0;
     if (const char* e = getenv("FY_PANEL_REPAIR")) t.panel_repair = atoi(e) != 0;
     if (const char* e = getenv("FY_PANEL_MULTI_LAUNCH")) t.panel_multi_launch = atoi(e) != 0;
     if (const char* e = getenv("FY_FLAT")) t.flat_batch = atoi(e) != 0;
diff --git a/filmyou-core_amd/csrc/fy_rm2.hip b/filmyou-core_amd/csrc/fy_rm2.hip
--- a/filmyou-core_amd/csrc/fy_rm2.hip
+++ b/filmyou-core_amd/csrc/fy_rm2.hip
@@ -1140,7 +1140,7 @@
     if (top_n_hint > TOPN_LONG) k_topn_long<<<n_rows, 256, (size_t)fy_topn_long_cap(top_n_hint) * 8, st>>>(TA, overflow, any_overflow, 0, fy_topn_long_cap(top_n_hint));
     else k_topn_fast<<<n_rows, 256, 0, st>>>(TA, overflow, any_overflow, 0);
     FY_KERNEL_CHECK();
-    k_topn_select<<<n_rows, 256, 0, st>>>(TA, overflow, any_overflow);
+    k_topn_select<<<fy_topn_select_grid(n_rows, ctx->num_cus), 256, 0, st>>>(TA, overflow, any_overflow, n_rows);
     FY_KERNEL_CHECK();
 }
 
@@ -2081,7 +2081,8 @@
                 const size_t ss = X.t_score->begin(st);
                 k_count_heavy_multi<<<(ny + 63) / 64, 64, 0, st>>>(F.d_flat[f].get(), (int32_t)ny);
                 FY_KERNEL_CHECK();
-                if (f) k_score_multi<4, true, 8><<<dim3((unsigned)max_grid[f], ny), 256, 0, st>>>(F.d_flat[f].get(), P.csr_idx.get(), X.csr_e, X.csr_q, X.pvpi, X.n_out);
+                if (f && tune.score_walk) k_score_multi<4, true, 8, 1><<<dim3((unsigned)max_grid[f], ny), 256, 0, st>>>(F.d_flat[f].get(), P.csr_idx.get(), X.csr_e, X.csr_q, X.pvpi, X.n_out);
+                else if (f) k_score_multi<4, true, 8, 0><<<dim3((unsigned)max_grid[f], ny), 256, 0, st>>>(F.d_flat[f].get(), P.csr_idx.get(), X.csr_e, X.csr_q, X.pvpi, X.n_out);
                 else k_score_multi<4, false, 8><<<dim3((unsigned)max_grid[f], ny), 256, 0, st>>>(F.d_flat[f].get(), P.csr_idx.get(), X.csr_e, X.csr_q, X.pvpi, X.n_out);
                 FY_KERNEL_CHECK();
                 X.t_score->end(ss, st);
@@ -2407,7 +2408,8 @@
         const int n_slices = score_slices(ctx->num_cus, tune, nb, n_chunks);
         ScoreArgs SA = score_args(L.M.get(), ldm, Ic, X.a_rank + pbase, s0, nb, Sx, ldS, n_slices, n_chunks);
         const size_t ss = X.t_score->begin(ls);
-        if (pack24) k_score<4, true, 8><<<n_chunks * n_slices, 256, 0, ls>>>(SA.M, SA.a_rank, SA.rb_off, SA.csr_idx, SA.csr_e, SA.csr_q, SA.pvpi, SA.n_out, SA.S, SA);
+        if (pack24 && tune.score_walk) k_score<4, true, 8, 1><<<n_chunks * n_slices, 256, 0, ls>>>(SA.M, SA.a_rank, SA.rb_off, SA.csr_idx, SA.csr_e, SA.csr_q, SA.pvpi, SA.n_out, SA.S, SA);
+        else if (pack24) k_score<4, true, 8, 0><<<n_chunks * n_slices, 256, 0, ls>>>(SA.M, SA.a_rank, SA.rb_off, SA.csr_idx, SA.csr_e, SA.csr_q, SA.pvpi, SA.n_out, SA.S, SA);
         else k_score<4, false, 8><<<n_chunks * n_slices, 256, 0, ls>>>(SA.M, SA.a_rank, SA.rb_off, SA.csr_idx, SA.csr_e, SA.csr_q, SA.pvpi, SA.n_out, SA.S, SA);
         FY_KERNEL_CHECK();
         X.t_score->end(ss, ls);
@@ -2421,7 +2423,7 @@
                                                                                                  fy_topn_long_cap(prm.number_of_recommendations));
         else k_topn_fast<<<nb, 256, 0, ls>>>(TA, L.overflow.get(), L.any_overflow.get(), tune.force_select);
         FY_KERNEL_CHECK();
-        k_topn_select<<<nb, 256, 0, ls>>>(TA, L.overflow.get(), L.any_overflow.get(), X.prune_counters + 2);
+        k_topn_select<<<fy_topn_select_grid(nb, ctx->num_cus), 256, 0, ls>>>(TA, L.overflow.get(), L.any_overflow.get(), nb, X.prune_counters + 2);
         FY_KERNEL_CHECK();
         X.t_topn->end(tt, ls);
         refine_rows(s0, nb);
@@ -2448,7 +2450,8 @@
             L.UBs.alloc(ctx, (size_t)nb * 64);
             SU.Bsup = L.Bsup.get(); SU.asup = L.asup.get(); SU.bsup_b = L.bsupb.get(); SU.UBsup = L.UBs.get();
             SU.n_sup = std::min(64, std::max(0, p.nblk - seed_chunks));
-            k_score_sup<<<seed_chunks * n_slices, 256, 0, ls>>>(SU.M, SU.a_rank, SU.rb_off, SU.csr_idx, SU.csr_e, SU.csr_q, SU.pvpi, SU.n_out, SU.S, SU);
+            if (tune.score_walk) k_score_sup<1><<<seed_chunks * n_slices, 256, 0, ls>>>(SU.M, SU.a_rank, SU.rb_off, SU.csr_idx, SU.csr_e, SU.csr_q, SU.pvpi, SU.n_out, SU.S, SU);
+            else k_score_sup<0><<<seed_chunks * n_slices, 256, 0, ls>>>(SU.M, SU.a_rank, SU.rb_off, SU.csr_idx, SU.csr_e, SU.csr_q, SU.pvpi, SU.n_out, SU.S, SU);
             FY_KERNEL_CHECK();
         }
         ScoreArgs SA = score_args(Gmat, gld, Ic, X.a_rank + pbase, s0, nb, L.S.get(), SC, n_slices, seed_chunks + bchunks);
@@ -2462,7 +2465,8 @@
         SA.ldS2 = bld;
         SA.no_mask2 = 1;
         if (!use_sup) {
-            k_score<4, true, 8><<<(seed_chunks + bchunks) * n_slices, 256, 0, ls>>>(SA.M, SA.a_rank, SA.rb_off, SA.csr_idx, SA.csr_e, SA.csr_q, SA.pvpi, SA.n_out, SA.S, SA);
+            if (tune.score_walk) k_score<4, true, 8, 1><<<(seed_chunks + bchunks) * n_slices, 256, 0, ls>>>(SA.M, SA.a_rank, SA.rb_off, SA.csr_idx, SA.csr_e, SA.csr_q, SA.pvpi, SA.n_out, SA.S, SA);
+            else k_score<4, true, 8, 0><<<(seed_chunks + bchunks) * n_slices, 256, 0, ls>>>(SA.M, SA.a_rank, SA.rb_off, SA.csr_idx, SA.csr_e, SA.csr_q, SA.pvpi, SA.n_out, SA.S, SA);
             FY_KERNEL_CHECK();
         }
         TopNArgs T1{L.S.get(), SC, Ic, X.n_out, X.out_off, P.rank_item_raw.get() + pbase, P.slot2du.get(), P.uid.get(),
@@ -2566,7 +2570,10 @@
         if (n_surv_total > 0) {
             ScoreArgs SQ = score_args(Gmat, gld, Ic, X.a_rank + pbase, s0, nb, L.Ssurv.get(), 0, n_slices, n_chunks);
             const int panel_blocks = p.panel ? p.panel_cols / 256 : 0x7FFFFFFF;
-            k_score_blocks<8><<<std::min(n_surv_total, ctx->num_cus * 16), 256, 0, ls>>>(SQ.M, SQ.a_rank, P.rowptr.get(), SQ.csr_idx, SQ.csr_e, SQ.csr_q, SQ.pvpi,
+            if (tune.score_walk) k_score_blocks<8, 1><<<std::min(n_surv_total, ctx->num_cus * 16), 256, 0, ls>>>(SQ.M, SQ.a_rank, P.rowptr.get(), SQ.csr_idx, SQ.csr_e, SQ.csr_q, SQ.pvpi,
+                                                                L.quad_prefix.get(), L.surv.get(), SQ.S, SQ, bld, X.prune_counters, panel_blocks,
+                                                                p.panel ? L.surv_mask.get() : nullptr);
+            else k_score_blocks<8, 0><<<std::min(n_surv_total, ctx->num_cus * 16), 256, 0, ls>>>(SQ.M, SQ.a_rank, P.rowptr.get(), SQ.csr_idx, SQ.csr_e, SQ.csr_q, SQ.pvpi,
                                                                 L.quad_prefix.get(), L.surv.get(), SQ.S, SQ, bld, X.prune_counters, panel_blocks,
                                                                 p.panel ? L.surv_mask.get() : nullptr);
             FY_KERNEL_CHECK();
@@ -2603,7 +2610,7 @@
                                                                                                  fy_topn_long_cap(prm.number_of_recommendations));
         else k_topn_fast<<<nb, 256, 0, ls>>>(TA, L.overflow.get(), L.any_overflow.get(), tune.force_select);
         FY_KERNEL_CHECK();
-        k_topn_select<<<nb, 256, 0, ls>>>(TA, L.overflow.get(), L.any_overflow.get(), X.prune_counters + 2);
+        k_topn_select<<<fy_topn_select_grid(nb, ctx->num_cus), 256, 0, ls>>>(TA, L.overflow.get(), L.any_overflow.get(), nb, X.prune_counters + 2);
         FY_KERNEL_CHECK();
         X.t_topn->end(tt, ls);
         refine_rows(s0, nb);
diff --git a/filmyou-core_amd/csrc/fy_rm2_coop.hpp b/filmyou-core_amd/csrc/fy_rm2_coop.hpp
--- a/filmyou-core_amd/csrc/fy_rm2_coop.hpp
+++ b/filmyou-core_amd/csrc/fy_rm2_coop.hpp
@@ -150,7 +150,8 @@
         SA.S2 = ub_send.get() + (int64_t)k * Umax * ldb;
         SA.ldS2 = ldb;
         SA.no_mask2 = 1;
-        k_score<4, true, 8><<<(seed_chunks + bchunks) * ns, 256, 0, ls>>>(SA.M, SA.a_rank, SA.rb_off, SA.csr_idx, SA.csr_e, SA.csr_q, SA.pvpi, SA.n_out, SA.S, SA);
+        if (tune.score_walk) k_score<4, true, 8, 1><<<(seed_chunks + bchunks) * ns, 256, 0, ls>>>(SA.M, SA.a_rank, SA.rb_off, SA.csr_idx, SA.csr_e, SA.csr_q, SA.pvpi, SA.n_out, SA.S, SA);
+        else k_score<4, true, 8, 0><<<(seed_chunks + bchunks) * ns, 256, 0, ls>>>(SA.M, SA.a_rank, SA.rb_off, SA.csr_idx, SA.csr_e, SA.csr_q, SA.pvpi, SA.n_out, SA.S, SA);
         FY_KERNEL_CHECK();
         R->st.score_launches += 2;
     }
@@ -214,7 +215,7 @@
         FY_HIP(hipMemsetAsync(any_overflow.get(), 0, sizeof(int32_t), ls));
         k_topn_fast<<<n_mine, 256, 0, ls>>>(TA, overflow.get(), any_overflow.get(), tune.force_select);
         FY_KERNEL_CHECK();
-        k_topn_select<<<n_mine, 256, 0, ls>>>(TA, overflow.get(), any_overflow.get(), X.prune_counters + 2);
+        k_topn_select<<<fy_topn_select_grid(n_mine, ctx->num_cus), 256, 0, ls>>>(TA, overflow.get(), any_overflow.get(), n_mine, X.prune_counters + 2);
         FY_KERNEL_CHECK();
         X.t_topn->end(tt, ls);
     }
diff --git a/filmyou-core_amd/csrc/fy_rm2_kernels.hpp b/filmyou-core_amd/csrc/fy_rm2_kernels.hpp
--- a/filmyou-core_amd/csrc/fy_rm2_kernels.hpp
+++ b/filmyou-core_amd/csrc/fy_rm2_kernels.hpp
@@ -71,6 +71,112 @@
     f[3] = __uint_as_float(__builtin_amdgcn_perm(0u, d.c, 0x0302010cu) >> (8 - FY_P24_SHIFT));
 }
 
+typedef float fy_v2f __attribute__((ext_vector_type(2)));
+typedef const __attribute__((address_space(1))) unsigned char* fy_gbytes;
+typedef const __attribute__((address_space(1))) uint32_t* fy_gwords;
+__device__ __forceinline__ fy_gbytes fy_row_base(const void* M, int j, uint32_t pitch) {
+    const unsigned long long rb = (unsigned long long)M + (unsigned long long)(uint32_t)j * (unsigned long long)pitch;
+    const unsigned long long rs = ((unsigned long long)(uint32_t)__builtin_amdgcn_readfirstlane((int)(rb >> 32)) << 32) |
+                                  (uint32_t)__builtin_amdgcn_readfirstlane((int)(uint32_t)rb);
+    return reinterpret_cast<fy_gbytes>(rs);
+}
+__device__ __forceinline__ unsigned fy_rated_mask(const int32_t* __restrict__ csr_idx_, int beg, int end, int row_mul, int row_add, int col0,
+                                                  unsigned* bm, int lane) {
+    if (lane < 8) bm[lane] = 0u;
+    __builtin_amdgcn_fence(__ATOMIC_ACQ_REL, "wavefront");
+    for (int k0 = beg; k0 < end; k0 += 64) {
+        const int k = k0 + lane;
+        if (k < end) {
+            const unsigned d = (unsigned)(csr_idx_[k] * row_mul + row_add - col0);
+            if (d < 256u) atomicOr(&bm[d >> 5], 1u << (d & 31u));
+        }
+    }
+    __builtin_amdgcn_fence(__ATOMIC_ACQ_REL, "wavefront");
+    const unsigned m = (bm[lane >> 3] >> ((lane & 7) * 4)) & 15u;
+    __builtin_amdgcn_fence(__ATOMIC_ACQ_REL, "wavefront");
+    return m;
+}
+template <bool SUP>
+__device__ __forceinline__ void fy_batch8_p24(const void* M, uint32_t pitch, uint32_t lane_off, bool live, const int (&jj)[8],
+                                              const float (&e)[8], const float (&qq)[8], fy_v2f a01, fy_v2f a23, fy_v2f b01, fy_v2f b23,
+                                              double* t, bool sup_here, const void* Bsup, uint32_t sup_off, float as_, float bs_, double& ts) {
+    U3 g[8];
+    float gs[SUP ? 8 : 1];
+#pragma unroll
+    for (int r = 0; r < 8; r++) g[r] = U3{0u, 0u, 0u};
+    if (live) {
+#pragma unroll
+        for (int r = 0; r < 8; r++) {
+            const fy_gwords gw = reinterpret_cast<fy_gwords>(fy_row_base(M, jj[r], pitch) + lane_off);
+            g[r].a = gw[0]; g[r].b = gw[1]; g[r].c = gw[2];
+        }
+    }
+    if constexpr (SUP) {
+        if (sup_here) {
+#pragma unroll
+            for (int r = 0; r < 8; r++) gs[r] = __uint_as_float(*reinterpret_cast<fy_gwords>(fy_row_base(Bsup, jj[r], 256u) + sup_off));
+        }
+    }
+    fy_v2f p01 = fy_v2f{1.f, 1.f}, p23 = fy_v2f{1.f, 1.f};
+    int pe[4] = {0, 0, 0, 0};
+    float ps = 1.f;
+    int pes = 0;
+#pragma unroll
+    for (int r = 0; r < 8; r++) {
+        if constexpr (SUP) {
+            if (sup_here) fy_logprod_step(fmaf(qq[r], bs_, fmaf(as_, e[r], gs[r])), ps, pes);
+        }
+        float gv[4];
+        fy_unpack24(g[r], gv);
+        const fy_v2f e2 = fy_v2f{e[r], e[r]}, q2 = fy_v2f{qq[r], qq[r]};
+        const fy_v2f x01 = __builtin_elementwise_fma(q2, b01, __builtin_elementwise_fma(a01, e2, fy_v2f{gv[0], gv[1]}));
+        const fy_v2f x23 = __builtin_elementwise_fma(q2, b23, __builtin_elementwise_fma(a23, e2, fy_v2f{gv[2], gv[3]}));
+        p01 *= fy_v2f{__builtin_amdgcn_frexp_mantf(x01.x), __builtin_amdgcn_frexp_mantf(x01.y)};
+        p23 *= fy_v2f{__builtin_amdgcn_frexp_mantf(x23.x), __builtin_amdgcn_frexp_mantf(x23.y)};
+        pe[0] += __builtin_amdgcn_frexp_expf(x01.x);
+        pe[1] += __builtin_amdgcn_frexp_expf(x01.y);
+        pe[2] += __builtin_amdgcn_frexp_expf(x23.x);
+        pe[3] += __builtin_amdgcn_frexp_expf(x23.y);
+    }
+    t[0] += fy_logprod_fold(p01.x, pe[0]);
+    t[1] += fy_logprod_fold(p01.y, pe[1]);
+    t[2] += fy_logprod_fold(p23.x, pe[2]);
+    t[3] += fy_logprod_fold(p23.y, pe[3]);
+    if constexpr (SUP) {
+        if (sup_here) ts += fy_logprod_fold(ps, pes);
+    }
+}
+template <bool SUP>
+__device__ __forceinline__ int fy_walk_full_p24(const void* M, uint32_t pitch, uint32_t lane_off, bool live, const int32_t* __restrict__ csr_idx_,
+                                                const float* __restrict__ csr_e_, const float* __restrict__ csr_q_, int beg, int end, fy_v2f a01,
+                                                fy_v2f a23, fy_v2f b01, fy_v2f b23, double* t, bool sup_here, const void* Bsup, uint32_t sup_off,
+                                                float as_, float bs_, double& ts) {
+    int k = __builtin_amdgcn_readfirstlane(beg);
+    end = __builtin_amdgcn_readfirstlane(end);
+    if (k + 8 > end) return k;
+    typedef const __attribute__((address_space(4))) int32_t* cints;
+    typedef const __attribute__((address_space(4))) float* cfloats;
+    const cints ci = reinterpret_cast<cints>(reinterpret_cast<unsigned long long>(csr_idx_));
+    const cfloats ce = reinterpret_cast<cfloats>(reinterpret_cast<unsigned long long>(csr_e_));
+    const cfloats cq = reinterpret_cast<cfloats>(reinterpret_cast<unsigned long long>(csr_q_));
+    int jj[8], jn[8];
+    float e[8], en[8], qq[8], qn[8];
+#pragma unroll
+    for (int r = 0; r < 8; r++) { jj[r] = ci[k + r]; e[r] = ce[k + r]; qq[r] = cq[k + r]; }
+    for (;;) {
+        const bool more = k + 16 <= end;
+        if (more) {
+#pragma unroll
+            for (int r = 0; r < 8; r++) { jn[r] = ci[k + 8 + r]; en[r] = ce[k + 8 + r]; qn[r] = cq[k + 8 + r]; }
+        }
+        fy_batch8_p24<SUP>(M, pitch, lane_off, live, jj, e, qq, a01, a23, b01, b23, t, sup_here, Bsup, sup_off, as_, bs_, ts);
+        k += 8;
+        if (!more) break;
+        for (int r = 0; r < 8; r++) { jj[r] = jn[r]; e[r] = en[r]; qq[r] = qn[r]; }
+    }
+    return k;
+}
+
 __device__ __forceinline__ bool fy_bound_keeps(float ub, float tau, float pvpi) {
     if (!(ub == ub) || tau == INFINITY) return false;
     if (tau == -INFINITY) return true;
@@ -78,7 +184,7 @@
     return ub + (4e-6f * S + 1e-4f) >= tau;
 }
 
-template <int VEC, bool P24, int SB, bool SUP = false>
+template <int VEC, bool P24, int SB, bool SUP = false, int WALK = 0>
 __device__ __forceinline__ void score_body(const float* __restrict__ M_, const float* __restrict__ a_rank_,
                                            const int32_t* __restrict__ rb_off_, const int32_t* __restrict__ csr_idx_,
                                            const float* __restrict__ csr_e_, const float* __restrict__ csr_q_,
@@ -87,6 +193,7 @@
     using V = typename VecT<VEC>::type;
     using G = typename std::conditional<P24, U3, V>::type;
     static_assert(!P24 || VEC == 4, "24-bit rows are packed four columns to three dwords");
+    static_assert(WALK == 0 || (P24 && SB == 8), "the second walk is that of the 24-bit rows, in batches of eight");
     constexpr int CW = 64 * VEC;
     const int lane = threadIdx.x & 63;
     const int wave = __builtin_amdgcn_readfirstlane(threadIdx.x >> 6);
@@ -119,7 +226,7 @@
     const double LN2 = 0.69314718055994530942;
     const float qnan = __builtin_nanf("");
     const int row_mul = A.row_mul ? A.row_mul : 1;
-    auto walk = [&](int beg, int end, double* t, unsigned& mask, double& ts) __attribute__((always_inline)) {
+    auto walk = [&](int beg, int end, double* t, unsigned& mask, double& ts, const bool do_mask) __attribute__((always_inline)) {
         if (beg >= end) return;
         static_assert(SB <= 64, "one lane per row of a batch");
         const int sub = lane & (SB - 1);
@@ -170,7 +277,7 @@
 #pragma unroll
                     for (int v = 0; v < VEC; v++) fy_logprod_step(fmaf(qq[q], bb[v], fmaf(a[v], e[q], gv[v])), p[v], pe[v]);
                     const unsigned d = (unsigned)(jj[q] * row_mul + A.row_add - col0);
-                    if (!no_mask && d < (unsigned)CW && (int)(d / VEC) == lane) mask |= 1u << (d % VEC);
+                    if (do_mask && !no_mask && d < (unsigned)CW && (int)(d / VEC) == lane) mask |= 1u << (d % VEC);
                 }
             }
 #pragma unroll
@@ -179,6 +286,20 @@
                 if (sup_here) ts += fy_logprod_fold(ps, pes);
             }
             vi = vi_n; ve = ve_n; vq = vq_n;
+        }
+    };
+    __shared__ unsigned sh_bm[WALK ? 4 : 1][8];
+    auto walk_rows = [&](int beg, int end, double* t, unsigned& mask, double& ts) __attribute__((always_inline)) {
+        if constexpr (WALK == 0) walk(beg, end, t, mask, ts, true);
+        else {
+            if (beg >= end) return;
+            if (!no_mask) mask |= fy_rated_mask(csr_idx_, beg, end, row_mul, A.row_add, col0, sh_bm[wave], lane);
+            fy_v2f a01, a23, b01, b23;
+            a01.x = a[0]; a01.y = a[1]; a23.x = a[2]; a23.y = a[3];
+            b01.x = bb[0]; b01.y = bb[1]; b23.x = bb[2]; b23.y = bb[3];
+            const int k = fy_walk_full_p24<SUP>(Msel, (uint32_t)pitch, (uint32_t)col * 3u, true, csr_idx_, csr_e_, csr_q_, beg, end, a01, a23, b01, b23, t,
+                                                sup_here, A.Bsup, (uint32_t)lane * 4u, as_, bs_, ts);
+            walk(k, end, t, mask, ts, false);
         }
     };
     auto store = [&](int u, int slot, const double* t, unsigned mask) __attribute__((always_inline)) {
@@ -213,7 +334,7 @@
         for (int v = 0; v < VEC; v++) t[v] = 0.0;
         unsigned mask = 0;
         double ts = 0.0;
-        walk(wb, we, t, mask, ts);
+        walk_rows(wb, we, t, mask, ts);
         if (wave > 0) {
 #pragma unroll
             for (int v = 0; v < VEC; v++) sh_t[wave - 1][lane][v] = t[v];
@@ -243,26 +364,27 @@
         for (int v = 0; v < VEC; v++) t[v] = 0.0;
         unsigned mask = 0;
         double ts = 0.0;
-        walk(beg, end, t, mask, ts);
+        walk_rows(beg, end, t, mask, ts);
         store(u, slot, t, mask);
         store_sup(u, slot, ts);
     }
 }
-template <int VEC, bool P24, int SB>
+template <int VEC, bool P24, int SB, int WALK = 0>
 __global__ __launch_bounds__(256) void k_score(const float* __restrict__ M_, const float* __restrict__ a_rank_,
                                                const int32_t* __restrict__ rb_off_, const int32_t* __restrict__ csr_idx_,
                                                const float* __restrict__ csr_e_, const float* __restrict__ csr_q_,
                                                const double* __restrict__ pvpi_,
                                                const int32_t* __restrict__ n_out_, float* __restrict__ S_, ScoreArgs A) {
-    score_body<VEC, P24, SB>(M_, a_rank_, rb_off_, csr_idx_, csr_e_, csr_q_, pvpi_, n_out_, S_, A, (int)blockIdx.x);
-}
-
+    score_body<VEC, P24, SB, false, WALK>(M_, a_rank_, rb_off_, csr_idx_, csr_e_, csr_q_, pvpi_, n_out_, S_, A, (int)blockIdx.x);
+}
+
+template <int WALK>
 __global__ __launch_bounds__(256) void k_score_sup(const float* __restrict__ M_, const float* __restrict__ a_rank_,
                                                    const int32_t* __restrict__ rb_off_, const int32_t* __restrict__ csr_idx_,
                                                    const float* __restrict__ csr_e_, const float* __restrict__ csr_q_,
                                                    const double* __restrict__ pvpi_,
                                                    const int32_t* __restrict__ n_out_, float* __restrict__ S_, ScoreArgs A) {
-    score_body<4, true, 8, true>(M_, a_rank_, rb_off_, csr_idx_, csr_e_, csr_q_, pvpi_, n_out_, S_, A, (int)blockIdx.x);
+    score_body<4, true, 8, true, WALK>(M_, a_rank_, rb_off_, csr_idx_, csr_e_, csr_q_, pvpi_, n_out_, S_, A, (int)blockIdx.x);
 }
 
 struct TopNArgs {
@@ -827,9 +949,15 @@
         A.out_cluster[off + i] = A.cluster;
     }
 }
+inline int fy_topn_select_grid(int n_rows, int num_cus) { return n_rows < 2 * num_cus ? n_rows : 2 * num_cus; }
 __global__ __launch_bounds__(256) void k_topn_select(TopNArgs A, const int32_t* __restrict__ overflow,
-                                                     const int32_t* __restrict__ any_overflow, unsigned long long* __restrict__ n_selected = nullptr) {
-    topn_select_body(A, overflow, any_overflow, n_selected, (int)blockIdx.x);
+                                                     const int32_t* __restrict__ any_overflow, int n_rows,
+                                                     unsigned long long* __restrict__ n_selected = nullptr) {
+    if (*any_overflow == 0) return;
+    for (int u = (int)blockIdx.x; u < n_rows; u += (int)gridDim.x) {
+        topn_select_body(A, overflow, any_overflow, n_selected, u);
+        __syncthreads();
+    }
 }
 
 struct FlatDesc {
@@ -850,14 +978,14 @@
     *d.n_heavy = lo;
     *d.any_overflow = 0;
 }
-template <int VEC, bool P24, int SB>
+template <int VEC, bool P24, int SB, int WALK = 0>
 __global__ __launch_bounds__(256) void k_score_multi(const FlatDesc* __restrict__ D, const int32_t* __restrict__ csr_idx_,
                                                      const float* __restrict__ csr_e_, const float* __restrict__ csr_q_,
                                                      const double* __restrict__ pvpi_, const int32_t* __restrict__ n_out_) {
     const FlatDesc& d = D[blockIdx.y];
     if ((int)blockIdx.x >= d.score_grid) return;
     const ScoreArgs A = d.SA;
-    score_body<VEC, P24, SB>(A.M, A.a_rank, A.rb_off, csr_idx_, csr_e_, csr_q_, pvpi_, n_out_, A.S, A, (int)blockIdx.x);
+    score_body<VEC, P24, SB, false, WALK>(A.M, A.a_rank, A.rb_off, csr_idx_, csr_e_, csr_q_, pvpi_, n_out_, A.S, A, (int)blockIdx.x);
 }
 __global__ __launch_bounds__(256) void k_topn_fast_multi(const FlatDesc* __restrict__ D, int force_select) {
     const FlatDesc& d = D[blockIdx.y];
@@ -884,7 +1012,7 @@
     }
 }
 
-template <int SB>
+template <int SB, int WALK = 0>
 __global__ __launch_bounds__(256) void k_score_blocks(const float* __restrict__ M_, const float* __restrict__ a_rank_,
                                                       const int32_t* __restrict__ rowptr_, const int32_t* __restrict__ csr_idx_,
                                                       const float* __restrict__ csr_e_, const float* __restrict__ csr_q_,
@@ -895,6 +1023,8 @@
                                                       const uint8_t* __restrict__ surv_mask_ = nullptr) {
     __shared__ double sh_t[3][64][4];
     __shared__ unsigned sh_mask[3][64];
+    __shared__ unsigned sh_bm[WALK ? 4 : 1][8];
+    static_assert(WALK == 0 || SB == 8, "the second walk runs in batches of eight");
     const int lane = threadIdx.x & 63;
     const int wave = __builtin_amdgcn_readfirstlane((int)(threadIdx.x >> 6));
     const int total = surv_prefix_[A.n_users];
@@ -925,9 +1055,21 @@
         const char* __restrict__ Mcol = reinterpret_cast<const char*>(M_) + (int64_t)col * 3;
         const int row_beg = rowptr_[slot], row_end = rowptr_[slot + 1];
         const int quarter = (((row_end - row_beg + 3) >> 2) + SB - 1) / SB * SB;
-        const int beg = min(row_end, row_beg + wave * quarter), end = min(row_end, beg + quarter);
+        int beg = min(row_end, row_beg + wave * quarter);
+        const int end = min(row_end, beg + quarter);
         double t[4] = {0.0, 0.0, 0.0, 0.0};
         unsigned mask = 0;
+        if constexpr (WALK != 0) {
+            if (beg < end) {
+                mask = fy_rated_mask(csr_idx_, beg, end, 1, 0, col0, sh_bm[wave], lane);
+                fy_v2f a01, a23, b01, b23;
+                a01.x = a[0]; a01.y = a[1]; a23.x = a[2]; a23.y = a[3];
+                b01.x = bb[0]; b01.y = bb[1]; b23.x = bb[2]; b23.y = bb[3];
+                double ts_unused = 0.0;
+                beg = fy_walk_full_p24<false>(M_, (uint32_t)pitch, (uint32_t)col * 3u, live, csr_idx_, csr_e_, csr_q_, beg, end, a01, a23, b01, b23, t, false,
+                                              nullptr, 0u, 0.f, 0.f, ts_unused);
+            }
+        }
         const int sub = lane & (SB - 1);
         int vi = 0, vi_n;
         float ve = 0.f, vq = 0.f, ve_n, vq_n;
@@ -961,7 +1103,7 @@
 #pragma unroll
                     for (int v = 0; v < 4; v++) fy_logprod_step(fmaf(qq[x], bb[v], fmaf(a[v], e[x], gv[v])), p[v], pe[v]);
                     const unsigned d = (unsigned)(jj[x] - col);
-                    if (d < 4u) mask |= 1u << d;
+                    if (WALK == 0 && d < 4u) mask |= 1u << d;
                 }
             }
 #pragma unroll
diff --git a/filmyou-core_amd/csrc/fy_tuning.hpp b/filmyou-core_amd/csrc/fy_tuning.hpp
--- a/filmyou-core_amd/csrc/fy_tuning.hpp
+++ b/filmyou-core_amd/csrc/fy_tuning.hpp
@@ -40,6 +40,7 @@
     bool bounded_tables = true;
     bool cooc_planes = true;
     int score_heavy = 512;
+    int score_walk = 1;
     bool panel_repair = true;
     int panel_lanes = 2;
     int64_t flat_budget = 0;
```

Result: faster. 404.3 million (median of 6 runs) (+1.7%).
